# spiraldb/vortex

Hardware: AMD Instinct MI355X
Metric: decoded GB/s/GPU (device-resident) per encoding; % HBM roofline (higher is better)
Workload: dtype u32

## Files before the change

### vortex_amd/arrays.py

```python
from __future__ import annotations

import ctypes as C
from dataclasses import dataclass, field
from typing import Any, Optional, Sequence

import numpy as np

from . import _lib
from ._lib import DTYPE, ENC, PTYPE, PTYPES, VALIDITY, VortexGpuError

NP_OF_PTYPE = {"u8": np.uint8, "u16": np.uint16, "u32": np.uint32, "u64": np.uint64,
               "i8": np.int8, "i16": np.int16, "i32": np.int32, "i64": np.int64,
               "f16": np.float16, "f32": np.float32, "f64": np.float64}
PTYPE_OF_NP = {np.dtype(v): k for k, v in NP_OF_PTYPE.items()}


def ptype_width(p: str) -> int:
    return np.dtype(NP_OF_PTYPE[p]).itemsize


def unsigned_of(p: str) -> str:
    return "u" + p[1:] if p[0] == "i" else p


# ... 131 lines not shown
    return Array(ENC["ZIGZAG"], encoded.len, DTYPE["PRIMITIVE"], "i" + encoded.ptype[1:],
                 encoded.nullable, VALIDITY["NON_NULLABLE"], {}, [], [encoded])


def alp(encoded: Array, e: int, f: int, patches: Optional[Array] = None) -> Array:
    fp = {"i32": "f32", "i64": "f64"}.get(encoded.ptype)
    if fp is None:
        _bail("MismatchedTypes", f"ALP encoded child must be i32/i64, got {encoded.ptype}")
    return Array(ENC["ALP"], encoded.len, DTYPE["PRIMITIVE"], fp, encoded.nullable,
                 VALIDITY["NON_NULLABLE"], {"e": e, "f": f, "has_patches": patches is not None},
                 [], [encoded] + ([patches] if patches is not None else []))


def alp_rd(ptype: str, left_parts: Array, left_dict: Sequence[int], right_parts: Array,
           right_bit_width: int, exceptions: Optional[Array] = None) -> Array:
    if left_parts.len != right_parts.len:
        _bail("InvalidArgument", "left_parts and right_parts must be of same length")
    if left_parts.ptype[0] != "u":
        _bail("InvalidArgument", "left_parts dtype must be uint")
    if right_parts.nullable or right_parts.ptype[0] != "u":
        _bail("MismatchedTypes", "right_parts must be non-nullable uint")
    d = list(left_dict) + [0] * (8 - len(left_dict))
    return Array(ENC["ALP_RD"], left_parts.len, DTYPE["PRIMITIVE"], ptype, left_parts.nullable,
                 VALIDITY["NON_NULLABLE"],
                 {"right_bit_width": right_bit_width, "dict_len": len(left_dict), "dict": d,
                  "left_parts_ptype": PTYPE[left_parts.ptype], "has_exceptions": exceptions is not None},
                 [], [left_parts, right_parts] + ([exceptions] if exceptions is not None else []))


def dict_array(values: Array, codes: Array) -> Array:
    if codes.ptype[0] != "u" or codes.nullable:
        _bail("MismatchedTypes", f"non-nullable unsigned int, got {codes.ptype}")
    return Array(ENC["DICT"], codes.len, values.dtype, values.ptype, values.nullable,
                 VALIDITY["NON_NULLABLE"], {"codes_ptype": PTYPE[codes.ptype], "values_len": values.len},
                 [], [values, codes])


def delta(bases: Array, deltas: Array, offset: int = 0, length: Optional[int] = None,
          validity=None) -> Array:
    length = deltas.len - offset if length is None else length
    if offset >= 1024:
        _bail("InvalidArgument", f"offset must be less than 1024: {offset}")
    if offset + length > deltas.len:
        _bail("InvalidArgument", "offset + logical_len must be <= the size of deltas")
    if bases.ptype != deltas.ptype:
        _bail("InvalidArgument", "DeltaArray: bases and deltas must have the same dtype")
    lanes = 1024 // (8 * ptype_width(deltas.ptype))
    expect = (deltas.len // 1024) * lanes + (1 if deltas.len % 1024 else 0)
    if bases.len != expect:
        _bail("InvalidArgument", f"DeltaArray: bases.len() ({bases.len}) != expected_bases_len ({expect})")
    nullable = validity is not None
    vk, vchild = _validity_kind(nullable, validity)
    return Array(ENC["FL_DELTA"], length, DTYPE["PRIMITIVE"], deltas.ptype, nullable, vk,
                 {"deltas_len": deltas.len, "offset": offset}, [],
                 [bases, deltas] + ([vchild] if vchild is not None else []))


def run_end(ends: Array, values: Array, length: Optional[int] = None, offset: int = 0,
            validity=None) -> Array:
    if ends.ptype[0] not in "ui":
        _bail("InvalidArgument", "Run ends must be integers")
    if ends.encoding == ENC["PRIMITIVE"] and ends.len:
        ev = np.asarray(ends.buffers[0]).view(NP_OF_PTYPE[ends.ptype])
        if length is None:
            length = int(ev[ends.len - 1])
        if offset != 0 and int(ev[0]) <= offset:
            _bail("InvalidArgument", f"First run end {int(ev[0])} must be bigger than offset {offset}")
    elif length is None and ends.len == 0:
        length = 0
    if length is None:
        _bail("InvalidArgument", "length needed for compressed ends")
    nullable = validity is not None
    vk, vchild = _validity_kind(nullable, validity)
    return Array(ENC["RUN_END"], length, DTYPE["PRIMITIVE"], values.ptype, nullable, vk,
                 {"ends_ptype": PTYPE[ends.ptype], "num_runs": ends.len, "offset": offset}, [],
                 [ends, values] + ([vchild] if vchild is not None else []))


def bool_array(mask, validity=None, bit_offset: int = 0) -> Array:
    m = np.asarray(mask, dtype=bool)
    bits = np.packbits(np.concatenate([np.zeros(bit_offset, bool), m]), bitorder="little")
    nullable = validity is not None
    vk, vchild = _validity_kind(nullable, validity)
    return Array(ENC["BOOL"], len(m), DTYPE["BOOL"], "u8", nullable, vk, {"first_byte_bit_offset": bit_offset},
                 [bits], [vchild] if vchild is not None else [])


def byte_bool(mask, validity=None) -> Array:
    b = np.asarray(mask).astype(np.uint8)
    nullable = validity is not None
    vk, vchild = _validity_kind(nullable, validity)
    return Array(ENC["BYTE_BOOL"], len(b), DTYPE["BOOL"], "u8", nullable, vk, {}, [b],
                 [vchild] if vchild is not None else [])


def roaring_bool(bitmap, length: int) -> Array:
    b = np.ascontiguousarray(bitmap).view(np.uint8).reshape(-1)
    return Array(ENC["ROARING_BOOL"], length, DTYPE["BOOL"], "u8", False, VALIDITY["NON_NULLABLE"], {}, [b])


def run_end_bool(ends: Array, start: bool, length: Optional[int] = None, offset: int = 0, validity=None) -> Array:
    if ends.ptype[0] != "u":
        _bail("InvalidArgument", f"Ends array must be an unsigned integer type, got {ends.ptype}")
    if ends.len == 0:
        _bail("InvalidArgument", "Ends array must have at least one element")
    if length is None:
        length = int(np.asarray(ends.buffers[0])[ends.len - 1]) if ends.encoding == ENC["PRIMITIVE"] else None
        if length is None:
            _bail("InvalidArgument", "length needed for compressed ends")
    nullable = validity is not None
    vk, vchild = _validity_kind(nullable, validity)
    return Array(ENC["RUN_END_BOOL"], length, DTYPE["BOOL"], "u8", nullable, vk,
                 {"start": bool(start), "ends_ptype": PTYPE[ends.ptype], "num_runs": ends.len, "offset": offset},
                 [], [ends] + ([vchild] if vchild is not None else []))


def constant_bool(value: Optional[bool], length: int) -> Array:
    sc = bytes(16) if value is None else bytes([1 if value else 0]).ljust(16, b"\0")
    return Array(ENC["CONSTANT"], length, DTYPE["BOOL"], "u8", value is None, VALIDITY["NON_NULLABLE"],
                 {"is_null": value is None, "scalar": sc})


def sparse_bool(indices: Array, values: Array, length: int, indices_offset: int = 0, fill=None) -> Array:
    if values.dtype != DTYPE["BOOL"]:
        _bail("MismatchedTypes", "sparse_bool values must be a Bool array")
    fill_bytes = bytes(16) if fill is None else bytes([1 if fill else 0]).ljust(16, b"\0")
    return Array(ENC["SPARSE"], length, DTYPE["BOOL"], "u8", True, VALIDITY["NON_NULLABLE"],
                 {"indices_offset": indices_offset, "indices_len": indices.len,
                  "fill_is_null": fill is None, "fill": fill_bytes}, [], [indices, values])


def constant(value, length: int, ptype: str) -> Array:
    sc = bytes(16) if value is None else np.array([value], dtype=NP_OF_PTYPE[ptype]).tobytes().ljust(16, b"\0")
    return Array(ENC["CONSTANT"], length, DTYPE["PRIMITIVE"], ptype, value is None,
                 VALIDITY["NON_NULLABLE"], {"is_null": value is None, "scalar": sc})


def chunked(chunks: Sequence[Array]) -> Array:
    if not chunks:
        _bail("InvalidArgument", "chunked needs at least one chunk for a dtype")
    d0 = (chunks[0].dtype, chunks[0].ptype)
    for c in chunks:
        if (c.dtype, c.ptype) != d0:
            _bail("MismatchedTypes", "Chunks must have the same dtype")
    offs = np.zeros(len(chunks) + 1, dtype=np.uint64)
    offs[1:] = np.cumsum([c.len for c in chunks])
    return Array(ENC["CHUNKED"], int(offs[-1]), chunks[0].dtype, chunks[0].ptype,
                 any(c.nullable for c in chunks), VALIDITY["NON_NULLABLE"],
                 {"nchunks": len(chunks)}, [], [primitive(offs)] + list(chunks))


def varbin(offsets: Array, data: Array, utf8: bool = True, validity=None) -> Array:
    nullable = validity is not None
    vk, vchild = _validity_kind(nullable, validity)
    return Array(ENC["VARBIN"], offsets.len - 1, DTYPE["UTF8" if utf8 else "BINARY"], "u8", nullable,
                 vk, {"offsets_ptype": PTYPE[offsets.ptype], "bytes_len": data.len}, [],
                 [offsets, data] + ([vchild] if vchild is not None else []))


def varbinview(views, buffers: Sequence, utf8: bool = True, validity=None) -> Array:
    v = np.ascontiguousarray(views, dtype=np.uint8).reshape(-1)
    if v.size % 16:
        _bail("InvalidArgument", "views must be a multiple of 16 bytes")
    bufs = [np.ascontiguousarray(b, dtype=np.uint8).reshape(-1) for b in buffers]
    if any(b.size >= 2 ** 32 for b in bufs):
        _bail("InvalidArgument", "buffer must be within 32-bit range")
    nullable = validity is not None
    vk, vchild = _validity_kind(nullable, validity)
    return Array(ENC["VARBINVIEW"], v.size // 16, DTYPE["UTF8" if utf8 else "BINARY"], "u8", nullable, vk,
                 {"n_buffers": len(bufs)}, [],
                 [primitive(v)] + [primitive(b) for b in bufs] + ([vchild] if vchild is not None else []))


def fsst(symbols: Array, symbol_lengths: Array, codes: Array, uncompressed_lengths: Array,
         utf8: bool = True) -> Array:
    if symbols.len > 255:
        _bail("InvalidArgument", "symbols array must have length <= 255")
    if symbols.len != symbol_lengths.len:
        _bail("InvalidArgument", "symbols and symbol_lengths arrays must have same length")
    if uncompressed_lengths.len != codes.len:
        _bail("InvalidArgument", "uncompressed_lengths must be same len as codes")
    if codes.encoding != ENC["VARBIN"]:
        _bail("InvalidArgument", "codes array must be VarBin")
    return Array(ENC["FSST"], codes.len, DTYPE["UTF8" if utf8 else "BINARY"], "u8", codes.nullable,
                 VALIDITY["NON_NULLABLE"],
                 {"symbols_len": symbols.len, "codes_nullable": codes.nullable,
                  "uncompressed_lengths_ptype": PTYPE[uncompressed_lengths.ptype]}, [],
                 [symbols, symbol_lengths, codes, uncompressed_lengths])


def _fill_meta(m: _lib.VxgMeta, a: Array) -> None:
    md = a.meta
    e = a.encoding
    if e == ENC["FL_BITPACKED"]:
        m.bitpacked.bit_width, m.bitpacked.has_patches, m.bitpacked.offset = (
            md["bit_width"], int(md["has_patches"]), md["offset"])
    elif e == ENC["FL_FOR"]:
        m.for_.reference, m.for_.shift = md["reference"], md["shift"]
    elif e == ENC["FL_DELTA"]:
        m.delta.deltas_len, m.delta.offset = md["deltas_len"], md["offset"]
    elif e == ENC["ALP"]:
        m.alp.e, m.alp.f, m.alp.has_patches = md["e"], md["f"], int(md["has_patches"])
    elif e == ENC["ALP_RD"]:
        m.alprd.right_bit_width = md["right_bit_width"]
        m.alprd.dict_len = md["dict_len"]
        m.alprd.left_parts_ptype = md["left_parts_ptype"]
        m.alprd.has_exceptions = int(md["has_exceptions"])
        for i, v in enumerate(md["dict"]):
            m.alprd.dict[i] = v
    elif e == ENC["DICT"]:
        m.dict.codes_ptype, m.dict.values_len = md["codes_ptype"], md["values_len"]
    elif e == ENC["FSST"]:
        m.fsst.symbols_len = md["symbols_len"]
        m.fsst.codes_nullable = int(md["codes_nullable"])
        m.fsst.uncompressed_lengths_ptype = md["uncompressed_lengths_ptype"]
    elif e == ENC["RUN_END"]:
        m.runend.ends_ptype, m.runend.num_runs, m.runend.offset = (
            md["ends_ptype"], md["num_runs"], md["offset"])
    elif e == ENC["SPARSE"]:
        m.sparse.indices_offset = md["indices_offset"]
        m.sparse.indices_len = md["indices_len"]
        m.sparse.fill_is_null = int(md["fill_is_null"])
        for i, b in enumerate(md["fill"][:16]):
            m.sparse.fill[i] = b
    elif e == ENC["CONSTANT"]:
        m.constant.is_null = int(md["is_null"])
        for i, b in enumerate(md["scalar"][:16]):
            m.constant.scalar[i] = b
    elif e == ENC["CHUNKED"]:
        m.chunked.nchunks = md["nchunks"]
    elif e == ENC["VARBIN"]:
        m.varbin.offsets_ptype, m.varbin.bytes_len = md["offsets_ptype"], md["bytes_len"]
    elif e == ENC["BOOL"]:
        m.boolean.first_byte_bit_offset = md.get("first_byte_bit_offset", 0)
    elif e == ENC["RUN_END_BOOL"]:
        m.runendbool.start, m.runendbool.ends_ptype = int(md["start"]), md["ends_ptype"]
        m.runendbool.num_runs, m.runendbool.offset = md["num_runs"], md["offset"]
    elif e == ENC["VARBINVIEW"]:
        m.varbinview.n_buffers = md["n_buffers"]


def _buf_ptr(b) -> tuple[int, int]:
    import torch
    if not isinstance(b, torch.Tensor) or not b.is_cuda:
        raise VortexError(3, "array buffers must be device tensors: call Array.to(device) first")
    return b.data_ptr(), b.numel() * b.element_size()


def flatten(a: Array, keep: list) -> _lib.VxgArray:
    node = _lib.VxgArray()
    node.encoding = a.encoding
    node.dtype = a.dtype
    node.ptype = PTYPE[a.ptype]
    node.nullable = int(a.nullable)
    node.validity = a.validity
    node.len = a.len
    _fill_meta(node.meta, a)
    if a.buffers:
        bufs = (_lib.VxgBuffer * len(a.buffers))()
        for i, b in enumerate(a.buffers):
            bufs[i].ptr, bufs[i].len = _buf_ptr(b)
            keep.append(b)
        keep.append(bufs)
        node.buffers = C.cast(bufs, C.POINTER(_lib.VxgBuffer))
        node.n_buffers = len(a.buffers)
    if a.children:
        kids = (_lib.VxgArray * len(a.children))()
        for i, c in enumerate(a.children):
            kids[i] = flatten(c, keep)
        keep.append(kids)
        node.children = C.cast(kids, C.POINTER(_lib.VxgArray))
        node.n_children = len(a.children)
    return node


class Context:

    def __init__(self, device: int = 0):
        self.lib = _lib.gpu_lib()
        self.device = device
        h = C.c_void_p()
        _lib.check(self.lib.vxg_open(device, C.byref(h)))
        self.handle = h

    def close(self):
        if self.handle:
            self.lib.vxg_close(self.handle)
            self.handle = None

    def __del__(self):
        try:
            self.close()
        except Exception:
            pass

    def stream_ptr(self):
        import torch
        return C.c_void_p(torch.cuda.current_stream(self.device).cuda_stream)

    def sync(self):
        _lib.check(self.lib.vxg_stream_sync(self.handle, self.stream_ptr()))

    _OPTIONS = {"k1w_min_groups": _lib.OPT_K1W_MIN_GROUPS, "k1w_bpw": _lib.OPT_K1W_BPW,
                "k1_wave": _lib.OPT_K1_WAVE}

    def set_option(self, name: str, value: int):
        _lib.check(self.lib.vxg_set_option(self.handle, self._OPTIONS[name], int(value)))

    def get_option(self, name: str) -> int:
        v = C.c_int64()
        _lib.check(self.lib.vxg_get_option(self.handle, self._OPTIONS[name], C.byref(v)))
        return v.value

    def launch_stats(self, reset: bool = False) -> dict:
        st = _lib.VxgLaunchStats()
        _lib.check(self.lib.vxg_get_launch_stats(self.handle, C.byref(st), int(reset)))
        return {f: getattr(st, f) for f, _ in st._fields_}


@dataclass
class Canonical:
    kind: str
    len: int
    ptype: str
    values: Any = None
    views: Any = None
    data: Any = None
    validity: Any = None
    data_buffers: Any = None
    binary: bool = False
    info: Any = None

    def to_arrow(self):
        import pyarrow as pa
        validity = None if self.validity is None else pa.py_buffer(self.validity.cpu().numpy()[: (self.len + 7) // 8].copy())
        nulls = -1 if validity is not None else 0
        if self.kind == "primitive":
            t = {"u8": pa.uint8(), "u16": pa.uint16(), "u32": pa.uint32(), "u64": pa.uint64(), "i8": pa.int8(),
                 "i16": pa.int16(), "i32": pa.int32(), "i64": pa.int64(), "f16": pa.float16(), "f32": pa.float32(),
                 "f64": pa.float64()}[self.ptype]
            return pa.Array.from_buffers(t, self.len, [validity, pa.py_buffer(self.values.cpu().numpy().copy())],
                                         null_count=nulls)
        if self.kind == "bool":
            bits = self.values.cpu().numpy()[: (self.len + 7) // 8].copy()
            return pa.Array.from_buffers(pa.bool_(), self.len, [validity, pa.py_buffer(bits)], null_count=nulls)
        data = self.data.cpu().numpy()
        bufs = [pa.py_buffer(data[o: o + n].copy()) for o, n in self.data_buffers]
        views = pa.py_buffer(self.views.cpu().numpy()[: 16 * self.len].copy())
        return pa.Array.from_buffers(pa.binary_view() if self.binary else pa.string_view(), self.len,
                                     [validity, views] + bufs, null_count=nulls)

    def numpy(self):
        if self.kind == "primitive":
            return self.values.cpu().numpy().view(NP_OF_PTYPE[self.ptype])
        if self.kind == "bool":
            return np.unpackbits(self.values.cpu().numpy(), bitorder="little")[: self.len].astype(bool)
        return self.views.cpu().numpy().reshape(-1, 16), self.data.cpu().numpy()

    def buffers(self):
        d = self.data.cpu().numpy()
        return [d[o: o + n] for o, n in self.data_buffers]

    def validity_mask(self):
        if self.validity is None:
            return None
        bits = self.validity.cpu().numpy()
        return np.unpackbits(bits, bitorder="little")[: self.len].astype(bool)


def _kind(a: Array) -> str:
    return {DTYPE["PRIMITIVE"]: "primitive", DTYPE["BOOL"]: "bool"}.get(a.dtype, "varbinview")


def canonicalize(a: Array, ctx: Context, out_values=None, sync: bool = True) -> Canonical:
    import torch
    keep: list = []
    node = flatten(a, keep)
    dev = torch.device("cuda", ctx.device)
    vb, db, nb = C.c_uint64(), C.c_uint64(), C.c_uint32()
    cap = 256
    while True:
        table = (_lib.VxgDataBuffer * cap)()
        st = ctx.lib.vxg_canonical_layout(ctx.handle, C.byref(node), C.byref(vb), C.byref(db), table, cap,
                                          C.byref(nb))
        if st == 3 and cap < (1 << 24):
            cap *= 16
            continue
        _lib.check(st)
        break
    out = _lib.VxgCanonical()
    res = Canonical(_kind(a), a.len, a.ptype, binary=a.dtype == DTYPE["BINARY"])
    nbits = ((a.len + 31) // 32) * 4
    valid_t = torch.empty(max(nbits, 4), dtype=torch.uint8, device=dev) if a.nullable else None
    if a.dtype in (DTYPE["PRIMITIVE"], DTYPE["BOOL"]):
        vals = out_values if out_values is not None else torch.empty(max(vb.value, 16), dtype=torch.uint8, device=dev)
        out.values = vals.data_ptr()
        res.values = vals[: vb.value]
    else:
        views = torch.empty(max(vb.value, 16), dtype=torch.uint8, device=dev)
        data = torch.empty(db.value + 16, dtype=torch.uint8, device=dev)
        out.views, out.data = views.data_ptr(), data.data_ptr()
        out.data_bytes = db.value
        out.data_buffers, out.n_data_buffers, out.data_buffers_cap = table, nb.value, nb.value
        res.views, res.data = views[: vb.value], data[: db.value]
        res.data_buffers = [(int(table[i].offset), int(table[i].len)) for i in range(nb.value)]
    if valid_t is not None:
        out.validity = valid_t.data_ptr()
    _lib.check(ctx.lib.vxg_canonicalize(ctx.handle, C.byref(node), C.byref(out), ctx.stream_ptr()))
    if out.validity:
        if valid_t is None or out.validity != valid_t.data_ptr():
            raise VortexError(7, "engine allocated validity for a non-nullable dtype")
        res.validity = valid_t[: (a.len + 7) // 8]
    if sync:
        ctx.sync()
    return res


def take(a: Array, indices, ctx: Context, sync: bool = True) -> Canonical:
    import torch
    keep: list = []
    node = flatten(a, keep)
    dev = torch.device("cuda", ctx.device)
    if isinstance(indices, torch.Tensor):
        it = indices.to(dev)
        tmap = {torch.uint8: "u8", torch.int8: "i8", torch.int16: "i16", torch.int32: "i32", torch.int64: "i64"}
        for name, p in (("uint16", "u16"), ("uint32", "u32"), ("uint64", "u64")):
            if hasattr(torch, name):
                tmap[getattr(torch, name)] = p
        if it.dtype not in tmap:
            raise VortexError(3, f"take: indices must be integers, got {it.dtype}")
        ip = tmap[it.dtype]
    else:
        ia = np.ascontiguousarray(indices)
        if ia.dtype not in PTYPE_OF_NP or ia.dtype.kind not in "iu":
            raise VortexError(3, f"take: indices must be integers, got {ia.dtype}")
        ip = PTYPE_OF_NP[ia.dtype]
        it = torch.from_numpy(ia.view(np.uint8).copy()).to(dev)
    n = int(it.numel() if isinstance(indices, torch.Tensor) else np.asarray(indices).size)
    out = _lib.VxgCanonical()
    w = ptype_width(a.ptype)
    vals = torch.empty(max(n * w, 16), dtype=torch.uint8, device=dev)
    out.values = vals.data_ptr()
    vt = torch.empty(((n + 31) // 32) * 4 + 4, dtype=torch.uint8, device=dev) if a.nullable else None
    if vt is not None:
        out.validity = vt.data_ptr()
    _lib.check(ctx.lib.vxg_take_array(ctx.handle, C.byref(node), PTYPE[ip], C.c_void_p(it.data_ptr()), n,
                                      C.byref(out), ctx.stream_ptr()))
    res = Canonical("primitive", n, a.ptype, values=vals[: n * w])
    if out.validity:
        if vt is None or out.validity != vt.data_ptr():
            raise VortexError(7, "engine allocated validity for a non-nullable dtype")
        res.validity = vt[: (n + 7) // 8]
    if sync:
        ctx.sync()
    return res


def filter(a: Array, predicate: Array, ctx: Context) -> Canonical:
    import torch
    keep: list = []
    node = flatten(a, keep)
    pnode = flatten(predicate, keep)
    dev = torch.device("cuda", ctx.device)
    n = a.len
    out = _lib.VxgCanonical()
    kind = _kind(a)
    if kind == "primitive":
        buf = torch.empty(max(n * ptype_width(a.ptype), 16), dtype=torch.uint8, device=dev)
        out.values = buf.data_ptr()
    elif kind == "bool":
        buf = torch.empty(((n + 31) // 32) * 4 + 4, dtype=torch.uint8, device=dev)
        out.values = buf.data_ptr()
    else:
        buf = torch.empty(max(16 * n, 16), dtype=torch.uint8, device=dev)
        out.views = buf.data_ptr()
    vt = torch.empty(((n + 31) // 32) * 4 + 4, dtype=torch.uint8, device=dev) if a.nullable else None
    if vt is not None:
        out.validity = vt.data_ptr()
    table = (_lib.VxgDataBuffer * 1)()
    out.data_buffers, out.data_buffers_cap = table, 1
    _lib.check(ctx.lib.vxg_filter_array(ctx.handle, C.byref(node), C.byref(pnode), C.byref(out), ctx.stream_ptr()))
    k = int(out.len)
    res = Canonical(kind, k, a.ptype, binary=a.dtype == DTYPE["BINARY"])
    if kind == "primitive":
        res.values = buf[: k * ptype_width(a.ptype)]
    elif kind == "bool":
        res.values = buf[: ((k + 31) // 32) * 4]
    else:
        res.views = buf[: 16 * k]
        hb = int(out.data_bytes)
        heap = torch.empty(hb + 16, dtype=torch.uint8, device=dev)
        if out.data:
            _lib.check(ctx.lib.vxg_memcpy_d2d(ctx.handle, C.c_void_p(heap.data_ptr()), C.c_void_p(out.data), hb,
                                              ctx.stream_ptr()))
            ctx.sync()
            _lib.check(ctx.lib.vxg_free(ctx.handle, C.c_void_p(out.data)))
        res.data = heap[:hb]
        res.data_buffers = [(0, hb)]
    if out.validity:
        if vt is None or out.validity != vt.data_ptr():
            raise VortexError(7, "engine allocated validity for a non-nullable dtype")
        res.validity = vt[: (k + 7) // 8]
    ctx.sync()
    return res


def compare(a: Array, op: str, scalar, ctx: Context, null_as_false: bool = False, sync: bool = True,
            out_values=None, out_validity=None) -> Canonical:
    import torch
    if op not in _lib.CMP_OP:
        raise VortexError(3, f"compare: unknown operator {op!r}")
    keep: list = []
    node = flatten(a, keep)
    dev = torch.device("cuda", ctx.device)
    nbytes = ((a.len + 63) // 64) * 8
    vals = out_values if out_values is not None else torch.empty(max(nbytes, 8), dtype=torch.uint8, device=dev)
    out = _lib.VxgCanonical()
    out.values = vals.data_ptr()
    vt = None
    if a.nullable and not null_as_false:
        vt = out_validity if out_validity is not None else torch.empty(max(nbytes, 8), dtype=torch.uint8, device=dev)
        out.validity = vt.data_ptr()
    flags = _lib.CMP_NULL_AS_FALSE if null_as_false else 0
    if a.dtype in (DTYPE["UTF8"], DTYPE["BINARY"]) and isinstance(scalar, (bytes, bytearray, memoryview, str)):
        sc = scalar.encode("utf-8") if isinstance(scalar, str) else bytes(scalar)
        sbuf = (C.c_uint8 * max(len(sc), 1)).from_buffer_copy(sc.ljust(1, b"\0"))
        info = _lib.VxgCompareBytesInfo()
        _lib.check(ctx.lib.vxg_compare_bytes(ctx.handle, C.byref(node), _lib.CMP_OP[op], sbuf, len(sc), flags,
                                             C.byref(out), C.byref(info), ctx.stream_ptr()))
    else:
        sc = np.array([scalar]).astype(NP_OF_PTYPE[a.ptype]).tobytes() if a.dtype == DTYPE["PRIMITIVE"] else bytes(8)
        sbuf = (C.c_uint8 * 8)(*sc.ljust(8, b"\0")[:8])
        info = _lib.VxgCompareInfo()
        _lib.check(ctx.lib.vxg_compare_scalar(ctx.handle, C.byref(node), _lib.CMP_OP[op], sbuf, flags, C.byref(out),
                                              C.byref(info), ctx.stream_ptr()))
    res = Canonical("bool", a.len, a.ptype, values=vals[:nbytes],
                    info={f: int(getattr(info, f)) for f, _ in info._fields_})
    if out.validity:
        if vt is None or out.validity != vt.data_ptr():
            raise VortexError(7, "engine allocated validity for a non-nullable dtype")
        res.validity = vt[:nbytes]
    if sync:
        ctx.sync()
    return res


def predicate_from(mask: Canonical) -> Array:
    if mask.kind != "bool":
        _bail("MismatchedTypes", "predicate_from needs a Bool canonical")
    if mask.validity is not None:
        _bail("InvalidArgument", "predicate must be non-nullable bool: compare with null_as_false=True")
    return Array(ENC["BOOL"], mask.len, DTYPE["BOOL"], "u8", False, VALIDITY["NON_NULLABLE"],
                 {"first_byte_bit_offset": 0}, [mask.values])


def _kind_of_node(node: _lib.VxgArray) -> str:
    return {DTYPE["PRIMITIVE"]: "primitive", DTYPE["BOOL"]: "bool"}.get(node.dtype, "varbinview")


def alloc_canonical(ctx: Context, node: _lib.VxgArray, keep: list, table_cap: int = 4096):
    import torch
    dev = torch.device("cuda", ctx.device)
    vb, db, nb = C.c_uint64(), C.c_uint64(), C.c_uint32()
    table = (_lib.VxgDataBuffer * table_cap)()
    _lib.check(ctx.lib.vxg_canonical_layout(ctx.handle, C.byref(node), C.byref(vb), C.byref(db), table,
                                            table_cap, C.byref(nb)))
    n = int(node.len)
    res = Canonical(_kind_of_node(node), n, PTYPES[node.ptype], binary=node.dtype == DTYPE["BINARY"])
    o = _lib.VxgCanonical()
    if node.dtype in (DTYPE["PRIMITIVE"], DTYPE["BOOL"]):
        vals = torch.empty(max(vb.value, 16), dtype=torch.uint8, device=dev)
        o.values = vals.data_ptr()
        res.values = vals[: vb.value]
    else:
        views = torch.empty(max(vb.value, 16), dtype=torch.uint8, device=dev)
        data = torch.empty(db.value + 16, dtype=torch.uint8, device=dev)
        o.views, o.data, o.data_bytes = views.data_ptr(), data.data_ptr(), db.value
        o.data_buffers, o.n_data_buffers, o.data_buffers_cap = table, nb.value, table_cap
        res.views, res.data = views[: vb.value], data[: db.value]
        res.data_buffers = [(int(table[k].offset), int(table[k].len)) for k in range(nb.value)]
        keep.append(table)
    if node.nullable:
        vt = torch.empty(((n + 31) // 32) * 4 + 4, dtype=torch.uint8, device=dev)
        o.validity = vt.data_ptr()
        res.validity = vt[: (n + 7) // 8]
    keep.append(res)
    return o, res


class Plan:

    def __init__(self, arrays: Sequence, ctx: Context, measure: bool = False):
        self.ctx = ctx
        self.keep: list = []
        n = len(arrays)
        self.nodes = (_lib.VxgArray * max(n, 1))()
        self.outs = (_lib.VxgCanonical * max(n, 1))()
        self.results = []
        for i, a in enumerate(arrays):
            self.nodes[i] = a if isinstance(a, _lib.VxgArray) else flatten(a, self.keep)
            o, res = alloc_canonical(ctx, self.nodes[i], self.keep)
            self.outs[i] = o
            self.results.append(res)
        h = C.c_void_p()
        flags = _lib.PLAN_MEASURE if measure else 0
        _lib.check(ctx.lib.vxg_plan_create_ex(ctx.handle, self.nodes, self.outs, n, flags, C.byref(h)))
        self.handle = h
# ... 32 lines not shown
```

### vortex_amd/csrc/capi.hip

```cpp
#include <algorithm>
#include <cstring>
#include <mutex>

#include "encode_gpu.hpp"
#include "planner.hpp"

namespace vxg {

const float kF10f[11] = {1.0f, 10.0f, 100.0f, 1000.0f, 10000.0f, 100000.0f, 1000000.0f,
                         10000000.0f, 100000000.0f, 1000000000.0f, 10000000000.0f};
const float kIF10f[11] = {1.0f, 0.1f, 0.01f, 0.001f, 0.0001f, 0.00001f, 0.000001f,
                          0.0000001f, 0.00000001f, 0.000000001f, 0.0000000001f};
const double kF10d[24] = {
    1.0, 10.0, 100.0, 1000.0, 10000.0, 100000.0, 1000000.0, 10000000.0, 100000000.0,
    1000000000.0, 10000000000.0, 100000000000.0, 1000000000000.0, 10000000000000.0,
    100000000000000.0, 1000000000000000.0, 10000000000000000.0, 100000000000000000.0,
    1000000000000000000.0, 10000000000000000000.0, 100000000000000000000.0,
    1000000000000000000000.0, 10000000000000000000000.0, 100000000000000000000000.0};
const double kIF10d[24] = {
    1.0, 0.1, 0.01, 0.001, 0.0001, 0.00001, 0.000001, 0.0000001, 0.00000001, 0.000000001,
    0.0000000001, 0.00000000001, 0.000000000001, 0.0000000000001, 0.00000000000001,
    0.000000000000001, 0.0000000000000001, 0.00000000000000001, 0.000000000000000001,
    0.0000000000000000001, 0.00000000000000000001, 0.000000000000000000001,
    0.0000000000000000000001, 0.00000000000000000000001};

static thread_local std::string g_last_error;

vxg_status set_error(vxg_status s, const std::string& msg) {
    if (s != VXG_OK) g_last_error = msg;
    return s;
}

vxg_status hip_check(hipError_t e, const char* what) {
    if (e == hipSuccess) return VXG_OK;
    return set_error(e == hipErrorOutOfMemory ? VXG_ERR_OUT_OF_MEMORY : VXG_ERR_HIP,
                     std::string(what) + ": " + hipGetErrorString(e));
}

thread_local Ctx* g_cur_ctx = nullptr;

Options default_options() {
    static const Options d = [] {
        Options o;
        o.k1w_min_groups = int64_t(env_int("VXG_K1W_MIN_GROUPS", INT64_MIN, INT64_MAX, o.k1w_min_groups));
        return o;
    }();
    return d;
}

vxg_status use_device(vxg_ctx* ctx) {
    if (!ctx) return set_error(VXG_ERR_INVALID_ARGUMENT, "null vxg_ctx");
    g_cur_ctx = &ctx->c;
    return hip_check(hipSetDevice(ctx->c.device), "hipSetDevice");
}

vxg_status status_of_err_word(uint32_t err) {
    if (err & kErrTakeOOB) return set_error(VXG_ERR_OUT_OF_BOUNDS, "take: index out of bounds");
    if (err & kErrPatchOOB) return set_error(VXG_ERR_OUT_OF_BOUNDS, "patch index out of bounds");
    if (err & kErrPatchOrder) return set_error(VXG_ERR_INVALID_ARGUMENT, "patch indices are not sorted");
    if (err & kErrRunEnd) return set_error(VXG_ERR_INVALID_ARGUMENT, "RunEnd ends do not cover the array");
    if (err & kErrFsst) return set_error(VXG_ERR_INVALID_ARGUMENT, "FSST codes do not decode to uncompressed_lengths");
    if (err & kErrRoaring) return set_error(VXG_ERR_INVALID_SERDE, "RoaringBool buffer is not a croaring Native bitmap");
    if (err & kErrVarBin) return set_error(VXG_ERR_INVALID_ARGUMENT, "VarBin offsets out of range of the bytes");
    if (err & kErrPlanSync)
        return set_error(VXG_ERR_ASSERTION_FAILED, "plan launch: in-grid pre-pass records never published "
                                                   "(overlapping replays of one plan?)");
    return set_error(VXG_ERR_ASSERTION_FAILED, "unknown device error bit");
}

}

using namespace vxg;

static vxg_status bitunpack_common(vxg_ctx* ctx, int T, unsigned W, unsigned offset, uint64_t len,
                                   const void* packed, uint64_t packed_bytes, Epi epi, int vw,
                                   UnpackArgs a, void* out, void* stream) {
    std::vector<K1Job> jobs(1);
    VXG_TRY(make_k1_job(T, W, offset, len, packed, packed_bytes, epi, vw, a, out, jobs[0]));
    return launch_k1_jobs(jobs, ctx->c.err_word, S(stream), nullptr, nullptr);
}

extern "C" {

int vxg_abi_version(void) { return VXG_ABI_VERSION; }

const char* vxg_last_error(void) { return g_last_error.c_str(); }

vxg_status vxg_open(int device, vxg_ctx** out) {
    if (!out) return set_error(VXG_ERR_INVALID_ARGUMENT, "null out");
    int n = 0;
    VXG_TRY(hip_check(hipGetDeviceCount(&n), "hipGetDeviceCount"));
    if (device < 0 || device >= n) return set_error(VXG_ERR_INVALID_ARGUMENT, "no such device");
    VXG_TRY(hip_check(hipSetDevice(device), "hipSetDevice"));
    auto* c = new vxg_ctx();
    c->c.device = device;
    c->c.opt = default_options();
    hipError_t e = hipMalloc(&c->c.err_word, 16);
    if (e == hipSuccess) e = hipMemset(c->c.err_word, 0, 16);
    if (e == hipSuccess) {
        hipMemPool_t pool;
        uint64_t keep = ~0ull;
        if (hipDeviceGetDefaultMemPool(&pool, device) == hipSuccess)
            (void)hipMemPoolSetAttribute(pool, hipMemPoolAttrReleaseThreshold, &keep);
    }
    if (e == hipSuccess) e = fsst_diag_init();
    if (e != hipSuccess) {
        vxg_close(c);
        return hip_check(e, "context setup");
    }
    *out = c;
    return VXG_OK;
}

vxg_status vxg_set_option(vxg_ctx* ctx, int option, int64_t value) {
    if (!ctx) return set_error(VXG_ERR_INVALID_ARGUMENT, "null vxg_ctx");
    Options& o = ctx->c.opt;
    switch (option) {
    case VXG_OPT_K1W_MIN_GROUPS:
        if (value < 0 || value > (int64_t(1) << 31)) return set_error(VXG_ERR_INVALID_ARGUMENT, "K1W_MIN_GROUPS out of range");
        o.k1w_min_groups = value;
        return VXG_OK;
    case VXG_OPT_K1W_BPW:
        if (value < 0 || value > 32) return set_error(VXG_ERR_INVALID_ARGUMENT, "K1W_BPW must be in [0, 32]");
        o.k1w_bpw = value;
        return VXG_OK;
    case VXG_OPT_K1_WAVE:
        if (value < -1 || value > 2) return set_error(VXG_ERR_INVALID_ARGUMENT, "K1_WAVE must be -1, 0, 1 or 2");
        o.k1_wave = value;
        return VXG_OK;
    }
    return set_error(VXG_ERR_INVALID_ARGUMENT, "unknown option " + std::to_string(option));
}

vxg_status vxg_get_option(vxg_ctx* ctx, int option, int64_t* value) {
    if (!ctx || !value) return set_error(VXG_ERR_INVALID_ARGUMENT, "null argument");
    const Options& o = ctx->c.opt;
    switch (option) {
    case VXG_OPT_K1W_MIN_GROUPS: *value = o.k1w_min_groups; return VXG_OK;
    case VXG_OPT_K1W_BPW: *value = o.k1w_bpw; return VXG_OK;
    case VXG_OPT_K1_WAVE: *value = o.k1_wave; return VXG_OK;
    }
    return set_error(VXG_ERR_INVALID_ARGUMENT, "unknown option " + std::to_string(option));
}

vxg_status vxg_get_launch_stats(vxg_ctx* ctx, vxg_launch_stats* out, int reset) {
    if (!ctx || !out) return set_error(VXG_ERR_INVALID_ARGUMENT, "null argument");
    std::lock_guard<std::mutex> lk(ctx->c.mu);
    const LaunchStats& st = ctx->c.st;
    *out = vxg_launch_stats{};
    out->k1w_launches = st.k1w_launches;
    out->k1w_last_groups = st.k1w_last_groups;
    out->k1w_last_bpw = st.k1w_last_bpw;
    out->k1w_min_bpw = st.k1w_min_bpw;
    out->k1w_max_bpw = st.k1w_max_bpw;
    out->k1w_last_bpw_max = st.k1w_last_bpw_max;
    if (reset) ctx->c.st = LaunchStats{};
    return VXG_OK;
}

vxg_status vxg_close(vxg_ctx* ctx) {
    if (!ctx) return VXG_OK;
    if (g_cur_ctx == &ctx->c) g_cur_ctx = nullptr;
    (void)hipSetDevice(ctx->c.device);
    (void)hipDeviceSynchronize();
    if (ctx->c.err_word) (void)hipFree(ctx->c.err_word);
    delete ctx;
    return VXG_OK;
}

vxg_status vxg_alloc(vxg_ctx* ctx, uint64_t bytes, void** dptr) {
    VXG_TRY(use_device(ctx));
    return hip_check(hipMalloc(dptr, bytes ? bytes : 16), "hipMalloc");
}

vxg_status vxg_free(vxg_ctx* ctx, void* dptr) {
    VXG_TRY(use_device(ctx));
    return hip_check(hipFree(dptr), "hipFree");
}

vxg_status vxg_host_alloc(vxg_ctx* ctx, uint64_t bytes, void** hptr) {
    VXG_TRY(use_device(ctx));
    return hip_check(hipHostMalloc(hptr, bytes ? bytes : 16, hipHostMallocDefault), "hipHostMalloc");
}

vxg_status vxg_host_free(vxg_ctx* ctx, void* hptr) {
    VXG_TRY(use_device(ctx));
    return hip_check(hipHostFree(hptr), "hipHostFree");
}

vxg_status vxg_memcpy_h2d(vxg_ctx* ctx, void* dst, const void* src, uint64_t bytes, void* stream) {
    VXG_TRY(use_device(ctx));
    return hip_check(hipMemcpyAsync(dst, src, bytes, hipMemcpyHostToDevice, S(stream)), "h2d");
}

vxg_status vxg_memcpy_d2h(vxg_ctx* ctx, void* dst, const void* src, uint64_t bytes, void* stream) {
    VXG_TRY(use_device(ctx));
    return hip_check(hipMemcpyAsync(dst, src, bytes, hipMemcpyDeviceToHost, S(stream)), "d2h");
}

vxg_status vxg_memcpy_d2d(vxg_ctx* ctx, void* dst, const void* src, uint64_t bytes, void* stream) {
    VXG_TRY(use_device(ctx));
    return hip_check(hipMemcpyAsync(dst, src, bytes, hipMemcpyDeviceToDevice, S(stream)), "d2d");
}

vxg_status vxg_stream_sync(vxg_ctx* ctx, void* stream) {
    VXG_TRY(use_device(ctx));
    VXG_TRY(hip_check(hipStreamSynchronize(S(stream)), "hipStreamSynchronize"));
    uint32_t err = 0;
    VXG_TRY(hip_check(hipMemcpy(&err, ctx->c.err_word, 4, hipMemcpyDeviceToHost), "error word readback"));
    if (err) {
        VXG_TRY(hip_check(hipMemset(ctx->c.err_word, 0, 4), "error word reset"));
        return status_of_err_word(err);
    }
    return VXG_OK;
}

vxg_status vxg_canonical_size(vxg_ctx* ctx, const vxg_array* a, uint64_t* values_bytes, uint64_t* data_bytes) {
    VXG_TRY(use_device(ctx));
    if (!a) return set_error(VXG_ERR_INVALID_ARGUMENT, "null array");
    Planner p(ctx, nullptr);
    uint64_t vb = 0, db = 0;
    VXG_TRY(p.canonical_size(*a, vb, db));
    if (values_bytes) *values_bytes = vb;
    if (data_bytes) *data_bytes = db;
    return VXG_OK;
}

vxg_status vxg_canonical_layout(vxg_ctx* ctx, const vxg_array* a, uint64_t* values_bytes, uint64_t* data_bytes,
                                vxg_data_buffer* bufs, uint32_t cap, uint32_t* n_bufs) {
    VXG_TRY(use_device(ctx));
    if (!a) return set_error(VXG_ERR_INVALID_ARGUMENT, "null array");
    Planner p(ctx, nullptr);
    uint64_t vb = 0, db = 0;
    uint32_t n = 0;
    if (is_string(*a)) {
        std::vector<vxg_data_buffer> v;
        VXG_TRY(p.string_layout(*a, v, db));
        vb = 16 * a->len;
        n = uint32_t(v.size());
        if (bufs && cap < n) return set_error(VXG_ERR_INVALID_ARGUMENT, "buffer table too small");
        if (bufs) std::copy(v.begin(), v.end(), bufs);
    } else {
        VXG_TRY(p.canonical_size(*a, vb, db));
    }
    if (values_bytes) *values_bytes = vb;
    if (data_bytes) *data_bytes = db;
    if (n_bufs) *n_bufs = n;
    return VXG_OK;
}

vxg_status vxg_canonicalize(vxg_ctx* ctx, const vxg_array* a, vxg_canonical* out, void* stream) {
    VXG_TRY(use_device(ctx));
    if (!a || !out) return set_error(VXG_ERR_INVALID_ARGUMENT, "null array/out");
    Planner p(ctx, S(stream));
    return p.canonical(*a, *out);
}

static int unsigned_T(int ptype) { return 8 * ptype_width(ptype); }

vxg_status vxg_bitunpack(vxg_ctx* ctx, int ptype, unsigned bit_width, unsigned offset, uint64_t len,
                         const void* packed, uint64_t packed_bytes, void* out, void* stream) {
    VXG_TRY(use_device(ctx));
    if (!ptype_is_int(ptype)) return set_error(VXG_ERR_MISMATCHED_TYPES, "BitPacked needs an integer ptype");
    return bitunpack_common(ctx, unsigned_T(ptype), bit_width, offset, len, packed, packed_bytes, Epi::Plain, 0,
                            UnpackArgs{}, out, stream);
}

vxg_status vxg_bitunpack_for(vxg_ctx* ctx, int ptype, unsigned bit_width, unsigned offset, uint64_t len,
                             const void* packed, uint64_t packed_bytes, uint64_t reference, unsigned shift,
                             int zigzag, void* out, void* stream) {
    VXG_TRY(use_device(ctx));
    if (!ptype_is_int(ptype)) return set_error(VXG_ERR_MISMATCHED_TYPES, "FoR needs an integer ptype");
    UnpackArgs a{};
    a.reference = reference;
    a.shift = shift;
    return bitunpack_common(ctx, unsigned_T(ptype), bit_width, offset, len, packed, packed_bytes,
                            zigzag ? Epi::ForZigZag : Epi::For, 0, a, out, stream);
}

vxg_status vxg_bitunpack_alp(vxg_ctx* ctx, int float_ptype, unsigned bit_width, unsigned offset, uint64_t len,
                             const void* packed, uint64_t packed_bytes, uint64_t for_reference,
                             unsigned for_shift, unsigned e, unsigned f, void* out, void* stream) {
    VXG_TRY(use_device(ctx));
    const bool f32 = float_ptype == VXG_F32;
    if (!f32 && float_ptype != VXG_F64) return set_error(VXG_ERR_MISMATCHED_TYPES, "ALP decodes to f32/f64");
    if ((f32 && (e > 10 || f > 10)) || (!f32 && (e > 23 || f > 23)))
        return set_error(VXG_ERR_INVALID_ARGUMENT, "ALP exponents out of range");
    UnpackArgs a{};
    a.reference = for_reference;
    a.shift = for_shift;
    a.alp_a = f32 ? double(kF10f[f]) : kF10d[f];
    a.alp_b = f32 ? double(kIF10f[e]) : kIF10d[e];
    return bitunpack_common(ctx, f32 ? 32 : 64, bit_width, offset, len, packed, packed_bytes,
                            f32 ? Epi::AlpF32 : Epi::AlpF64, 0, a, out, stream);
}

vxg_status vxg_bitunpack_dict(vxg_ctx* ctx, int codes_ptype, unsigned bit_width, unsigned offset, uint64_t len,
                              const void* packed, uint64_t packed_bytes, const void* dict_values,
                              uint64_t dict_len, unsigned value_width, void* out, void* stream) {
    VXG_TRY(use_device(ctx));
    if (!ptype_is_unsigned(codes_ptype)) return set_error(VXG_ERR_MISMATCHED_TYPES, "Dict codes must be unsigned");
    if (bit_width > unsigned(kDictFusedMaxW))
        return set_error(VXG_ERR_NOT_IMPLEMENTED, "fused dict decode supports code widths <= 16");
    UnpackArgs a{};
    a.dict = dict_values;
    a.dict_len = dict_len;
    return bitunpack_common(ctx, unsigned_T(codes_ptype), bit_width, offset, len, packed, packed_bytes, Epi::Dict,
                            int(value_width), a, out, stream);
}

vxg_status vxg_bitunpack_dict_chunks(vxg_ctx* ctx, int codes_ptype, unsigned bit_width, unsigned value_width,
                                     const vxg_dict_chunk* chunks_host, uint32_t n_chunks, void* stream) {
    VXG_TRY(use_device(ctx));
    if (!ptype_is_unsigned(codes_ptype)) return set_error(VXG_ERR_MISMATCHED_TYPES, "Dict codes must be unsigned");
    if (bit_width > unsigned(kDictFusedMaxW))
        return set_error(VXG_ERR_NOT_IMPLEMENTED, "fused dict decode supports code widths <= 16");
    std::vector<K1Job> jobs(n_chunks);
    for (uint32_t i = 0; i < n_chunks; i++) {
        const vxg_dict_chunk& c = chunks_host[i];
        if (c.n_blocks != (c.len + 1023) / 1024)
            return set_error(VXG_ERR_INVALID_ARGUMENT, "chunk n_blocks != ceil(len/1024)");
        UnpackArgs a{};
        a.dict = c.dict_values;
        a.dict_len = c.dict_len;
        VXG_TRY(make_k1_job(unsigned_T(codes_ptype), bit_width, 0, c.len, c.packed, c.n_blocks * 128ull * bit_width,
                            Epi::Dict, int(value_width), a, c.out, jobs[i]));
    }
    return launch_k1_jobs(jobs, ctx->c.err_word, S(stream), nullptr, nullptr);
}

vxg_status vxg_patch(vxg_ctx* ctx, int ptype, void* out, uint64_t out_len, int indices_ptype, const void* indices,
                     uint64_t indices_offset, const void* values, uint64_t n_patches, void* stream) {
    VXG_TRY(use_device(ctx));
    const int w = ptype_width(ptype);
    if (!w || !ptype_is_int(indices_ptype)) return set_error(VXG_ERR_INVALID_ARGUMENT, "bad ptype");
    UnpackArgs a{};
    a.err = ctx->c.err_word;
    IntCol ic{};
    ic.p = indices;
    ic.width = ptype_width(indices_ptype);
    ic.sgn = ptype_is_signed(indices_ptype);
    return launch_patch(0, ic, Epi::Plain, 8 * w, out, out_len, indices_offset, values, n_patches, a, S(stream));
}

vxg_status vxg_for_decode(vxg_ctx* ctx, int ptype, const void* in, uint64_t n, uint64_t reference,
                          unsigned shift, void* out, void* stream) {
    VXG_TRY(use_device(ctx));
    if (!ptype_is_int(ptype)) return set_error(VXG_ERR_MISMATCHED_TYPES, "FoR needs an integer ptype");
    return launch_for(ptype_width(ptype), in, n, reference, shift, false, out, S(stream));
}

vxg_status vxg_zigzag_decode(vxg_ctx* ctx, int out_ptype, const void* in, uint64_t n, void* out, void* stream) {
    VXG_TRY(use_device(ctx));
    if (!ptype_is_signed(out_ptype)) return set_error(VXG_ERR_MISMATCHED_TYPES, "ZigZag decodes to signed ints");
    return launch_zigzag(ptype_width(out_ptype), in, n, out, S(stream));
}

vxg_status vxg_alp_decode(vxg_ctx* ctx, int float_ptype, const void* encoded, uint64_t n, unsigned e, unsigned f,
                          void* out, void* stream) {
    VXG_TRY(use_device(ctx));
    const bool f32 = float_ptype == VXG_F32;
    if ((f32 && (e > 10 || f > 10)) || (!f32 && (e > 23 || f > 23)))
        return set_error(VXG_ERR_INVALID_ARGUMENT, "ALP exponents out of range");
    return launch_alp(float_ptype, encoded, n, f32 ? double(kF10f[f]) : kF10d[f],
                      f32 ? double(kIF10f[e]) : kIF10d[e], out, S(stream));
}

vxg_status vxg_alprd_decode(vxg_ctx* ctx, int float_ptype, const uint16_t* left_codes, const uint16_t* dict_host,
                            unsigned dict_len, unsigned right_bw, const void* right, uint64_t n,
                            const uint64_t* exc_pos, const uint16_t* exc_vals, uint64_t n_exc, void* out,
                            void* stream) {
    VXG_TRY(use_device(ctx));
    if (dict_len > 8) return set_error(VXG_ERR_INVALID_ARGUMENT, "ALP-RD dictionary holds at most 8 entries");
    return launch_alprd(float_ptype, left_codes, dict_host, dict_len, right_bw, right, n, exc_pos, 8, false, 0,
                        exc_vals, n_exc, out, ctx->c.err_word, S(stream));
}

vxg_status vxg_take(vxg_ctx* ctx, unsigned value_width, const void* values, uint64_t n_values, int codes_ptype,
                    const void* codes, uint64_t n, void* out, void* stream) {
    VXG_TRY(use_device(ctx));
    if (!ptype_is_unsigned(codes_ptype)) return set_error(VXG_ERR_MISMATCHED_TYPES, "take indices must be unsigned");
    return launch_take(int(value_width), values, n_values, ptype_width(codes_ptype), ptype_is_signed(codes_ptype), codes, n, out,
                       ctx->c.err_word, S(stream));
}

vxg_status vxg_delta_decode(vxg_ctx* ctx, int ptype, const void* bases, uint64_t n_bases, const void* deltas,
                            uint64_t n_deltas, uint64_t offset, uint64_t len, void* out, void* stream) {
    VXG_TRY(use_device(ctx));
    const int w = ptype_width(ptype);
    if (!ptype_is_unsigned(ptype)) return set_error(VXG_ERR_MISMATCHED_TYPES, "Delta decodes unsigned ints");
    const uint64_t lanes = 1024 / (8 * w);
    if (n_bases != (n_deltas / 1024) * lanes + (n_deltas % 1024 ? 1 : 0))
        return set_error(VXG_ERR_INVALID_ARGUMENT, "DeltaArray: bases.len() != expected_bases_len");
    if (offset + len > n_deltas) return set_error(VXG_ERR_INVALID_ARGUMENT, "offset + len > deltas len");
    return launch_delta(w, bases, deltas, n_deltas, offset, len, out, S(stream));
}

vxg_status vxg_runend_decode(vxg_ctx* ctx, unsigned value_width, const void* values, int ends_ptype,
                             const void* ends, uint64_t n_runs, uint64_t offset, uint64_t len, void* out,
                             void* stream) {
    VXG_TRY(use_device(ctx));
    if (!ptype_is_int(ends_ptype)) return set_error(VXG_ERR_MISMATCHED_TYPES, "RunEnd ends must be integers");
    RunEndChunk c{};
    c.ends.p = ends;
    c.ends.width = ptype_width(ends_ptype);
    c.ends.sgn = ptype_is_signed(ends_ptype);
    c.values.p = values;
    c.values.width = int(value_width);
    c.out = out;
    c.n_runs = n_runs;
    c.offset = offset;
    c.len = len;
    return launch_runend(int(value_width), c, ctx->c.err_word, S(stream));
}

vxg_status vxg_take_array(vxg_ctx* ctx, const vxg_array* a, int indices_ptype, const void* indices,
                          uint64_t n_indices, vxg_canonical* out, void* stream) {
    VXG_TRY(use_device(ctx));
    if (!a || !out || (n_indices && !indices)) return set_error(VXG_ERR_INVALID_ARGUMENT, "null array/indices/out");
    if (!ptype_is_int(indices_ptype)) return set_error(VXG_ERR_INVALID_ARGUMENT, "take indices must be integers");
    Planner p(ctx, S(stream));
    return p.take(*a, indices, ptype_width(indices_ptype), ptype_is_signed(indices_ptype), n_indices, *out);
}

vxg_status vxg_compare_scalar(vxg_ctx* ctx, const vxg_array* a, int op, const void* scalar_host, uint32_t flags,
                              vxg_canonical* out, vxg_compare_info* info, void* stream) {
    VXG_TRY(use_device(ctx));
    if (!a || !out || !scalar_host) return set_error(VXG_ERR_INVALID_ARGUMENT, "null array/scalar/out");
    uint64_t bits = 0;
    if (a->dtype == VXG_DTYPE_PRIMITIVE) std::memcpy(&bits, scalar_host, size_t(ptype_width(a->ptype)));
    vxg_compare_info ci{};
    Planner p(ctx, S(stream));
    void* const values_in = out->values;
    void* const validity_in = out->validity;
    const vxg_status st = p.compare(*a, op, bits, flags, *out, ci);
    if (info) *info = ci;
    if (st != VXG_OK) {
        if (out->values && out->values != values_in) (void)hipFree(out->values);
        if (out->validity && out->validity != validity_in) (void)hipFree(out->validity);
        out->values = values_in;
        out->validity = validity_in;
    }
    return st;
// ... 187 lines not shown
```

### vortex_amd/csrc/chunk_pack.hpp

```cpp
#pragma once

#include <algorithm>
#include <type_traits>

#include "vxg_internal.hpp"

namespace vxg {

template <class Tab, class It, class Entry, class Groups>
vxg_status pack_chunk_table(Tab& tab, It& it, It end, DevTables* dt, Entry entry, Groups groups_of, uint64_t* groups) {
    using E = std::remove_reference_t<decltype(tab.c[0])>;
    constexpr size_t cap = sizeof(tab.c) / sizeof(tab.c[0]);
    size_t take = 0;
    for (It k = it; k != end; ++k) take += entry(*k) != nullptr;
    E* cs = tab.c;
    if (dt && take > cap) {
        if (take > 0xFFFFFFFFull) return set_error(VXG_ERR_INVALID_ARGUMENT, "too many chunks");
        E* host;
        const vxg_status st = dt->table(take, &host, &tab.ext);
        if (st != VXG_OK) return st;
        if constexpr (requires { tab.host; }) tab.host = host;
        cs = host;
    } else {
        take = std::min(take, cap);
    }
    tab.n = 0;
    *groups = 0;
    for (; it != end && tab.n < take; ++it) {
        const E* e = entry(*it);
        if (!e) continue;
        E& c = cs[tab.n++];
        c = *e;
        c.first_group = *groups;
        *groups += groups_of(c);
    }
    while (it != end && !entry(*it)) ++it;
    if (*groups > 0xFFFFFFFFull) return set_error(VXG_ERR_INVALID_ARGUMENT, "array too long for one launch");
    return VXG_OK;
}

}
```

### vortex_amd/csrc/dict_rows.hip

```cpp
#include "fl_unpack_impl.hpp"

namespace vxg {

namespace {

constexpr int kRowsThreads = 256;
constexpr int kRowsMaxW = 16;

template <int VW> struct DVal;
template <> struct DVal<16> { using t = uint4; };

template <int T, int VW, int BPW, bool LDSD, bool EXT>
__global__ __launch_bounds__(kRowsThreads) void dict_rows_kernel(ChunkTable tab, unsigned W) {
    using E = typename Fl<T>::E;
    using V = typename DVal<VW>::t;
    constexpr unsigned LANES = 1024 / T;
    const uint64_t g = blockIdx.x;
    uint32_t ci;
    if constexpr (EXT) {
        ci = ext_chunk_index(tab.ext, tab.n, g, [](const ChunkDev& d) { return d.first_group; });
    } else {
        uint32_t lo = 0, hi = tab.n;
        while (hi - lo > 1) {
            const uint32_t mid = (lo + hi) >> 1;
            if (tab.c[mid].first_group <= g) lo = mid; else hi = mid;
        }
        ci = lo;
    }
    const ChunkDev& c = EXT ? tab.ext[ci] : tab.c[ci];
    __shared__ __attribute__((aligned(16))) E s_packed[BPW * 128 * kRowsMaxW / sizeof(E)];
    __shared__ __attribute__((aligned(16))) uint8_t s_dict[LDSD ? kDictLdsBytes : 16];
    const unsigned tid = threadIdx.x;
    const uint64_t blk0 = (g - c.first_group) * BPW;
    const unsigned nb = unsigned(c.n_blocks - blk0 < uint64_t(BPW) ? c.n_blocks - blk0 : uint64_t(BPW));
    const unsigned q16 = nb * 8 * W;
    for (unsigned q = tid; q < q16; q += kRowsThreads)
        reinterpret_cast<uint4*>(s_packed)[q] = reinterpret_cast<const uint4*>(c.packed + blk0 * (128ull * W))[q];
    const V* dict = static_cast<const V*>(c.dict);
    if constexpr (LDSD) {
        const unsigned n16 = unsigned((c.dict_len * VW + 15) / 16);
        for (unsigned q = tid; q < n16; q += kRowsThreads)
            reinterpret_cast<uint4*>(s_dict)[q] = static_cast<const uint4*>(c.dict)[q];
        dict = reinterpret_cast<const V*>(s_dict);
    }
    __syncthreads();
    V* __restrict__ out = static_cast<V*>(c.out);
    const RtRows<T> rows(W);
    bool oob = false;
    for (unsigned b = 0; b < nb; b++) {
        const E* __restrict__ pw = s_packed + b * (LANES * W);
        const int64_t base = int64_t((blk0 + b) * 1024) - int64_t(c.offset);
        const bool whole = base >= 0 && uint64_t(base) + 1024 <= c.len;
#pragma unroll
        for (unsigned k = 0; k < 4; k++) {
            const int64_t o = base + int64_t(k * kRowsThreads + tid);
            if (!whole && (o < 0 || uint64_t(o) >= c.len)) continue;
            const uint64_t code = W ? uint64_t(rows.get(pw, k)) : 0;
            const bool bad = code >= c.dict_len;
            oob |= bad;
            nt_store(out + o, dict[bad ? 0 : code]);
        }
    }
    if (oob) __hip_atomic_fetch_or(tab.err, kErrTakeOOB, __ATOMIC_RELAXED, __HIP_MEMORY_SCOPE_AGENT);
}

template <int T, int VW, int BPW, bool LDSD, bool EXT>
vxg_status launch_rows(ChunkTable tab, unsigned W, hipStream_t s) {
    ChunkDev* cs = tab.ext ? tab.host : tab.c;
    uint64_t groups = 0;
    for (uint32_t k = 0; k < tab.n; k++) {
        cs[k].first_group = groups;
        groups += (cs[k].n_blocks + BPW - 1) / BPW;
    }
    if (groups == 0) return VXG_OK;
    if (groups > 0xFFFFFFFFull) return set_error(VXG_ERR_INVALID_ARGUMENT, "array too long for one launch");
    hipLaunchKernelGGL((dict_rows_kernel<T, VW, BPW, LDSD, EXT>), dim3(unsigned(groups)), dim3(kRowsThreads), 0, s,
                       tab, W);
    return hip_check(hipGetLastError(), "dict_rows_kernel launch");
}

template <int T, int VW, int BPW>
vxg_status launch_rows_b(const ChunkTable& tab, unsigned W, bool lds, hipStream_t s) {
    if (tab.ext) return lds ? launch_rows<T, VW, BPW, true, true>(tab, W, s) : launch_rows<T, VW, BPW, false, true>(tab, W, s);
    return lds ? launch_rows<T, VW, BPW, true, false>(tab, W, s) : launch_rows<T, VW, BPW, false, false>(tab, W, s);
}

template <int T, int VW>
vxg_status launch_rows_t(const ChunkTable& tab, unsigned W, hipStream_t s) {
    const ChunkDev* cs = tab.ext ? tab.host : tab.c;
    bool lds = true;
    uint64_t max_dict = 0;
    for (uint32_t k = 0; k < tab.n; k++) {
        lds = lds && cs[k].dict_len * VW <= uint64_t(kDictLdsBytes) && (reinterpret_cast<uintptr_t>(cs[k].dict) & 15) == 0;
        max_dict = cs[k].dict_len * VW > max_dict ? cs[k].dict_len * VW : max_dict;
    }
    if (lds && max_dict > 1024) return launch_rows_b<T, VW, 8>(tab, W, lds, s);
    return launch_rows_b<T, VW, 1>(tab, W, lds, s);
}

}

vxg_status launch_dict_rows(int T, int W, const ChunkTable& tab, hipStream_t s) {
    if (W < 0 || W > kRowsMaxW || W > T) return VXG_ERR_NOT_IMPLEMENTED;
    const unsigned w = unsigned(W);
    switch (T) {
    case 8: return launch_rows_t<8, 16>(tab, w, s);
    case 16: return launch_rows_t<16, 16>(tab, w, s);
    case 32: return launch_rows_t<32, 16>(tab, w, s);
    case 64: return launch_rows_t<64, 16>(tab, w, s);
    }
    return VXG_ERR_NOT_IMPLEMENTED;
}

}
```

### vortex_amd/csrc/fl_unpack_impl.hpp

```cpp
#pragma once

#include <hip/hip_runtime.h>

#include <cstdint>
#include <cstdlib>
#include <type_traits>
#include <utility>

#include "vxg_internal.hpp"
#include "intcol.hpp"

namespace vxg {

template <int T> struct Fl;
template <> struct Fl<8> {
    using E = uint8_t;  using U = uint32_t;
    static constexpr uint32_t rep(uint32_t m) { return m * 0x01010101u; }
};
template <> struct Fl<16> {
    using E = uint16_t; using U = uint32_t;
    static constexpr uint32_t rep(uint32_t m) { return m * 0x00010001u; }
};
template <> struct Fl<32> {
    using E = uint32_t; using U = uint32_t;
// ... 284 lines not shown
    constexpr int WLO = W > 0 ? (R0 * W) / T : 0;
    constexpr int WHI = W > 0 ? (R1 * W - 1) / T : 0;
    Vec16<T> p[NW];
    if constexpr (W > 0) {
#pragma unroll
        for (int w = WLO; w <= WHI && w < W; w++) p[w] = load16<T>(blk_packed + 128 * w + 16 * t);
    }
    bool oob = false;
    if (full)
        process_rows_part<T, W, EPI, VW, NT, S, Q, true>(p, t * EPV, out, out_base, len, ep, oob,
                                                         std::make_integer_sequence<int, T / S>{});
    else
        process_rows_part<T, W, EPI, VW, NT, S, Q, false>(p, t * EPV, out, out_base, len, ep, oob,
                                                          std::make_integer_sequence<int, T / S>{});
    if constexpr (EPI == Epi::Dict)
        if (oob) __hip_atomic_fetch_or(ep.err, kErrTakeOOB, __ATOMIC_RELAXED, __HIP_MEMORY_SCOPE_AGENT);
}

constexpr int kDictLdsBytes = 16 * 1024;

template <int VW>
__device__ __forceinline__ void stage_dict(uint8_t* s_dict, const void* dict, uint64_t dict_len) {
    const int n16 = int((dict_len * VW + 15) / 16);
    for (int q = threadIdx.x; q < n16; q += blockDim.x)
        reinterpret_cast<uint4*>(s_dict)[q] = static_cast<const uint4*>(dict)[q];
    __syncthreads();
}

template <int T, int W, Epi EPI, int VW, bool LDSD, int S>
__device__ __forceinline__ void unpack_chunk(const ChunkDev& c, uint64_t g, uint32_t* err) {
    using O = typename EpiOut<T, EPI, VW>::type;
    constexpr int BPG = 32 / S;
    const uint64_t blk = (g - c.first_group) * BPG + ((threadIdx.x >> 3) % BPG);
    const int t = int(threadIdx.x & 7);
    EpiParams ep;
    ep.reference = c.reference;
    ep.shift = c.shift;
    ep.alp_a = c.alp_a;
    ep.alp_b = c.alp_b;
    ep.dict = c.dict;
    ep.dict_len = c.dict_len;
    ep.err = err;
    if constexpr (LDSD) {
        __shared__ __attribute__((aligned(16))) uint8_t s_dict[kDictLdsBytes];
        stage_dict<VW>(s_dict, c.dict, c.dict_len);
        ep.dict = s_dict;
        ep.dict_lds = true;
    }
    if (blk >= c.n_blocks) return;
    const int64_t out_base = int64_t(blk * 1024) - int64_t(c.offset);
    const bool full =
        c.offset == 0 && (blk + 1) * 1024 <= c.len && (reinterpret_cast<uintptr_t>(c.out) & 15) == 0;
    const uint8_t* bp = c.packed + blk * (128 * W);
    if constexpr (S == 1) {
        unpack_block<T, W, EPI, VW, kOutNT>(bp, t, static_cast<O*>(c.out), out_base, full, c.len, ep);
    } else {
        static_assert(S == 4, "row split 1 or 4");
        switch (threadIdx.x >> 6) {
        case 0: unpack_block_part<T, W, EPI, VW, kOutNT, 4, 0>(bp, t, static_cast<O*>(c.out), out_base, full, c.len, ep); break;
        case 1: unpack_block_part<T, W, EPI, VW, kOutNT, 4, 1>(bp, t, static_cast<O*>(c.out), out_base, full, c.len, ep); break;
        case 2: unpack_block_part<T, W, EPI, VW, kOutNT, 4, 2>(bp, t, static_cast<O*>(c.out), out_base, full, c.len, ep); break;
        default: unpack_block_part<T, W, EPI, VW, kOutNT, 4, 3>(bp, t, static_cast<O*>(c.out), out_base, full, c.len, ep); break;
        }
    }
}

constexpr int kw_bpw(int W, bool lds_dict = false) {
    const int b = ((lds_dict ? 16 : 32) * 1024) / (128 * (W > 0 ? W : 1));
    const int b4 = (b / 4) * 4;
    return b4 < 4 ? 4 : (b4 > 32 ? 32 : b4);
}

template <int T>
__device__ __forceinline__ int kw_row(int q) {
    constexpr int P = T / 8;
    const int s = q / P, f = (q % P) * (64 / T);
    const int o = ((f & 1) << 2) | (f & 2) | (f >> 2);
    return o * 8 + s;
}

template <typename U>
__device__ __forceinline__ U kw_mask(int n) {
    return n >= int(8 * sizeof(U)) ? ~U(0) : ((U(1) << n) - U(1));
}

template <int T, int W>
__device__ __forceinline__ Vec16<T> kw_extract(const uint8_t* blk, int r, int t) {
    using U = typename Fl<T>::U;
    constexpr int NV = Vec16<T>::NV;
    Vec16<T> v;
    if constexpr (W == 0) {
#pragma unroll
        for (int k = 0; k < NV; k++) v.w[k] = 0;
    } else {
        const int start = r * W, w0 = start / T, sh = start % T;
        const Vec16<T> lo = load16<T>(blk + w0 * 128 + 16 * t);
        if constexpr (W == T) {
            v = lo;
        } else {
            const Vec16<T> hi = load16<T>(blk + (w0 + 1) * 128 + 16 * t);
            const int cur = T - sh;
            const int nlo = cur < W ? cur : W, nhi = W - nlo;
            const U mlo = Fl<T>::rep(kw_mask<U>(nlo)), mhi = Fl<T>::rep(kw_mask<U>(nhi));
            const int hs = cur & (int(8 * sizeof(U)) - 1);
#pragma unroll
            for (int k = 0; k < NV; k++) v.w[k] = ((lo.w[k] >> sh) & mlo) | ((hi.w[k] & mhi) << hs);
        }
    }
    return v;
}

template <int T, int W, Epi EPI, int VW, int NT>
__device__ __forceinline__ void kw_block(const uint8_t* pk, int gq, int t, typename EpiOut<T, EPI, VW>::type* __restrict__ out,
                                         int64_t out_base, bool full, uint64_t len, const EpiParams& ep, bool& oob) {
    using E = typename Fl<T>::E;
    using O = typename EpiOut<T, EPI, VW>::type;
    constexpr int EPV = 16 / int(sizeof(E));
#pragma unroll
    for (int k = 0; k < T / 8; k++) {
        const int q = 8 * k + gq;
        const Vec16<T> v = kw_extract<T, W>(pk, kw_row<T>(q), t);
        const int idx = q * (1024 / T) + t * EPV;
        if (full) {
            O* dst = out + (out_base + idx);
            if constexpr (EPI == Epi::Plain) {
                store_bytes<16, NT>(reinterpret_cast<uint8_t*>(dst), v.w);
            } else {
                O o[EPV];
#pragma unroll
                for (int j = 0; j < EPV; j++) o[j] = apply_epi<T, EPI, VW>(v.elem(j), ep, oob);
                store_bytes<EPV * int(sizeof(O)), NT>(reinterpret_cast<uint8_t*>(dst), o);
            }
        } else {
#pragma unroll
            for (int j = 0; j < EPV; j++) {
                const int64_t o = out_base + idx + j;
                if (o >= 0 && uint64_t(o) < len) gstore(out + o, apply_epi<T, EPI, VW>(v.elem(j), ep, oob));
            }
        }
    }
}

template <int W, bool LDSD>
constexpr int kw_packed_lds() {
    return (W > 0 ? kw_bpw(W, LDSD) * 128 * W : 0) + 128;
}

__device__ __forceinline__ uint64_t patch_lower_bound(const PatchCol& pc, uint64_t x, uint32_t* s_cnt) {
    uint64_t lo = 0, hi = pc.n;
    while (lo < hi) {
        const uint64_t step = (hi - lo + 255) / 256;
        const uint64_t i = lo + uint64_t(threadIdx.x) * step;
        const bool below = i < hi && uint64_t(intcol_get(pc.idx, i)) - pc.idx_off < x;
        const uint32_t cw = uint32_t(__popcll(__ballot(below)));
        if ((threadIdx.x & 63) == 0) s_cnt[threadIdx.x >> 6] = cw;
        __syncthreads();
        const uint64_t cnt = uint64_t(s_cnt[0]) + s_cnt[1] + s_cnt[2] + s_cnt[3];
        __syncthreads();
        if (cnt == 0) {
            hi = lo;
        } else {
            const uint64_t nhi = lo + cnt * step;
            lo = lo + (cnt - 1) * step + 1;
            hi = nhi < hi ? nhi : hi;
        }
    }
    return lo;
}

template <int T, int W, Epi EPI, int VW, bool LDSD>
__device__ __forceinline__ void unpack_chunk_w(const ChunkDev& c, uint64_t g, uint32_t* err, const PatchCol& pc,
                                               uint32_t bpw_rt) {
    using O = typename EpiOut<T, EPI, VW>::type;
    constexpr int BPW_MAX = kw_bpw(W, LDSD);
    const int BPW = bpw_rt ? int(bpw_rt) : BPW_MAX;
    extern __shared__ __attribute__((aligned(16))) uint8_t k1w_lds[];
    uint8_t* const s_pk = k1w_lds;
    EpiParams ep;
    ep.reference = c.reference;
    ep.shift = c.shift;
    ep.alp_a = c.alp_a;
    ep.alp_b = c.alp_b;
    ep.dict = c.dict;
    ep.dict_len = c.dict_len;
    ep.err = err;
    if constexpr (LDSD) {
        uint8_t* const s_dict = k1w_lds + kw_packed_lds<W, LDSD>();
        stage_dict<VW>(s_dict, c.dict, c.dict_len);
        ep.dict = s_dict;
        ep.dict_lds = true;
    }
    const uint64_t blk0 = (g - c.first_group) * BPW;
    const int nb = c.n_blocks - blk0 < uint64_t(BPW) ? int(c.n_blocks - blk0) : BPW;
    uint32_t* const s_pscr = reinterpret_cast<uint32_t*>(k1w_lds + (W > 0 ? BPW * 128 * W : 0));
    const bool patched = pc.n != 0;
    uint64_t olo = 0, ohi = 0, pbase = 0, pw0 = 0, pw1 = 0;
    uint32_t psh = 0;
    O pval{};
    if (patched) {
        const uint64_t s0 = blk0 * 1024, s1 = (blk0 + uint64_t(nb)) * 1024;
        olo = s0 > c.offset ? s0 - c.offset : 0;
        ohi = s1 - c.offset < c.len ? s1 - c.offset : c.len;
        const uint64_t guess = uint64_t(double(olo) * double(pc.n) / double(c.len));
        pbase = guess > 128 ? guess - 128 : 0;
        if (pbase + 256 > pc.n) pbase = pc.n > 256 ? pc.n - 256 : 0;
        const uint64_t i0 = pbase + threadIdx.x, i = i0 < pc.n ? i0 : pc.n - 1;
        const uint64_t* ip = static_cast<const uint64_t*>(pc.idx.p);
        uint64_t a0 = i, a1 = i;
        if (pc.idx.packed) {
            const uint64_t g2 = i + pc.idx.offset;
            const uint32_t e = uint32_t(g2 & 1023), lane = e % 16, s = e >> 7;
            const uint32_t fl = ((e & 127) - lane) >> 4;
            const uint32_t row = (((fl & 1) << 2) | (fl & 2) | (fl >> 2)) * 8 + s;
            const uint32_t start = __umul24(row, pc.idx.W), word = start / 64;
            psh = start % 64;
            const uint64_t blk = (g2 >> 10) * (16ull * pc.idx.W);
            a0 = blk + 16ull * word + lane;
            a1 = blk + 16ull * (word + 1 < pc.idx.W ? word + 1 : word) + lane;
        }
        pw0 = ip[a0];
        pw1 = ip[a1];
        pval = static_cast<const O*>(pc.vals)[i];
    }
    if constexpr (W > 0) {
        using u32x4 = unsigned int __attribute__((ext_vector_type(4)));
        const gptr<const u32x4> src = (gptr<const u32x4>)(c.packed + blk0 * (128 * W));
#if VXG_K1W_BURST
        constexpr int NQ = BPW_MAX * 8 * W, PQ = (NQ + 255) / 256;
        if (nb == BPW_MAX) {
            u32x4 v[PQ];
#pragma unroll
            for (int p = 0; p < PQ; p++) {
                const int q = int(threadIdx.x) + 256 * p;
                v[p] = __builtin_nontemporal_load(src + (q < NQ ? q : NQ - 1));
            }
#pragma unroll
            for (int p = 0; p < PQ; p++) {
                const int q = int(threadIdx.x) + 256 * p;
                if (q < NQ) reinterpret_cast<uint4*>(s_pk)[q] = make_uint4(v[p][0], v[p][1], v[p][2], v[p][3]);
            }
        } else
#endif
        for (int q = threadIdx.x; q < nb * 8 * W; q += 256) {
            const u32x4 v = __builtin_nontemporal_load(src + q);
            reinterpret_cast<uint4*>(s_pk)[q] = make_uint4(v[0], v[1], v[2], v[3]);
        }
    }
    __syncthreads();
    const int wave = threadIdx.x >> 6, lane = threadIdx.x & 63, gq = lane >> 3, t = lane & 7;
    O* const out = static_cast<O*>(c.out);
    const bool aligned = (reinterpret_cast<uintptr_t>(c.out) & 15) == 0;
    bool oob = false;
    const int PER = (BPW + 3) / 4;
    for (int j = 0; j < PER; j++) {
        const int b = wave * PER + j;
        if (b >= nb) break;
        const uint64_t blk = blk0 + b;
        const int64_t out_base = int64_t(blk * 1024) - int64_t(c.offset);
        const bool full = c.offset == 0 && (blk + 1) * 1024 <= c.len && aligned;
        kw_block<T, W, EPI, VW, kOutNT>(s_pk + b * 128 * W, gq, t, out, out_base, full, c.len, ep, oob);
    }
    if constexpr (EPI == Epi::Dict)
        if (oob) __hip_atomic_fetch_or(err, kErrTakeOOB, __ATOMIC_RELAXED, __HIP_MEMORY_SCOPE_AGENT);
    if (patched) {
        asm volatile("" : "+v"(pw0), "+v"(pw1));
        uint64_t pkey = pw0;
        if (pc.idx.packed) {
            const uint64_t mask = pc.idx.W >= 64 ? ~0ull : ((1ull << pc.idx.W) - 1);
            const uint64_t v = pc.idx.W ? ((psh ? (pw0 >> psh) | (pw1 << (64 - psh)) : pw0) & mask) : 0;
            pkey = (v << pc.idx.shift) + pc.idx.reference;
        }
        const bool valid = pbase + threadIdx.x < pc.n;
        pkey = valid ? pkey - pc.idx_off : ~0ull;
        const bool pin = pkey >= olo && pkey < ohi;
        if (threadIdx.x == 0) s_pscr[0] = pbase == 0 || pkey < olo;
        if (threadIdx.x == 255) s_pscr[1] = pbase + 256 >= pc.n || pkey >= ohi;
        const uint64_t nk = __shfl_down(pkey, 1, 64);
        if ((threadIdx.x & 63) != 63 && pbase + threadIdx.x + 1 < pc.n && nk < pkey)
            __hip_atomic_fetch_or(err, kErrPatchOrder, __ATOMIC_RELAXED, __HIP_MEMORY_SCOPE_AGENT);
        if (g == c.first_group && threadIdx.x == 0) {
            const uint64_t k0 = uint64_t(intcol_get(pc.idx, 0)) - pc.idx_off;
            const uint64_t k1 = uint64_t(intcol_get(pc.idx, pc.n - 1)) - pc.idx_off;
            if (k0 >= c.len || k1 >= c.len)
                __hip_atomic_fetch_or(err, kErrPatchOOB, __ATOMIC_RELAXED, __HIP_MEMORY_SCOPE_AGENT);
        }
        __builtin_amdgcn_s_waitcnt(0);
        __syncthreads();
        if (s_pscr[0] && s_pscr[1]) {
            if (pin) gstore(out + pkey, pval);
        } else {
            const uint64_t ps = patch_lower_bound(pc, olo, s_pscr + 4);
            const uint64_t pe = patch_lower_bound(pc, ohi, s_pscr + 4);
            bool bad = false;
            for (uint64_t i = ps + threadIdx.x; i < pe; i += 256) {
                const uint64_t key = uint64_t(intcol_get(pc.idx, i)) - pc.idx_off;
                if (key >= olo && key < ohi) gstore(out + key, gload(static_cast<const O*>(pc.vals) + i));
                else bad = true;
            }
            if (bad) __hip_atomic_fetch_or(err, kErrPatchOrder, __ATOMIC_RELAXED, __HIP_MEMORY_SCOPE_AGENT);
        }
    }
}

template <int T, int W, Epi EPI, int VW, bool LDSD, bool EXT>
__global__ __launch_bounds__(256) void fl_unpack_w_kernel(ChunkTable tab) {
    const uint64_t g = blockIdx.x;
    if constexpr (EXT) {
        const ChunkDev& c =
            tab.ext[ext_chunk_index(tab.ext, tab.n, g, [](const ChunkDev& d) { return d.first_group; })];
        unpack_chunk_w<T, W, EPI, VW, LDSD>(c, g, tab.err, PatchCol{}, tab.bpw);
    } else {
        uint32_t lo = 0, hi = tab.n;
        while (hi - lo > 1) {
            const uint32_t mid = (lo + hi) >> 1;
            if (tab.c[mid].first_group <= g) lo = mid; else hi = mid;
        }
        unpack_chunk_w<T, W, EPI, VW, LDSD>(tab.c[lo], g, tab.err, tab.patch, tab.bpw);
    }
}

template <int T, int W, Epi EPI, int VW, bool LDSD = false, int S = 1, bool EXT = false>
__global__ __launch_bounds__(256) void fl_unpack_kernel(ChunkTable tab) {
    const uint64_t g = blockIdx.x;
    if constexpr (EXT) {
        const ChunkDev& c =
            tab.ext[ext_chunk_index(tab.ext, tab.n, g, [](const ChunkDev& d) { return d.first_group; })];
        unpack_chunk<T, W, EPI, VW, LDSD, S>(c, g, tab.err);
    } else {
        uint32_t lo = 0, hi = tab.n;
        while (hi - lo > 1) {
            const uint32_t mid = (lo + hi) >> 1;
            if (tab.c[mid].first_group <= g) lo = mid; else hi = mid;
        }
        unpack_chunk<T, W, EPI, VW, LDSD, S>(tab.c[lo], g, tab.err);
    }
}


inline int k1w_pick_bpw(uint64_t blocks, int bpw_max, int64_t min_groups, int64_t forced) {
    if (forced > 0) return int(forced < bpw_max ? forced : bpw_max);
    if (min_groups <= 0 || blocks >= uint64_t(min_groups) * uint64_t(bpw_max)) return bpw_max;
    const uint64_t b = blocks / uint64_t(min_groups);
    const int bpw = int(b < 4 ? 4 : (b / 4) * 4);
    return bpw > bpw_max ? bpw_max : bpw;
}

template <int T, int W, Epi EPI, int VW, bool LDSD, bool EXT>
vxg_status launch_w(ChunkTable tab, hipStream_t s) {
    constexpr int BPW_MAX = kw_bpw(W, LDSD);
    ChunkDev* cs = tab.ext ? tab.host : tab.c;
    uint64_t blocks = 0;
    for (uint32_t k = 0; k < tab.n; k++) blocks += cs[k].n_blocks;
    const Options o = cur_options();
    const int BPW = k1w_pick_bpw(blocks, BPW_MAX, o.k1w_min_groups, o.k1w_bpw);
    tab.bpw = uint32_t(BPW);
    uint64_t groups = 0, dict_bytes = 0;
    for (uint32_t k = 0; k < tab.n; k++) {
        cs[k].first_group = groups;
        groups += (cs[k].n_blocks + BPW - 1) / BPW;
        const uint64_t db = (cs[k].dict_len * uint64_t(VW > 0 ? VW : 1) + 15) & ~15ull;
        dict_bytes = db > dict_bytes ? db : dict_bytes;
    }
    if (groups == 0) return VXG_OK;
    if (groups > 0xFFFFFFFFull) return set_error(VXG_ERR_INVALID_ARGUMENT, "array too long for one launch");
    const size_t shm = LDSD ? size_t(kw_packed_lds<W, LDSD>()) + size_t(dict_bytes)
                            : size_t(W > 0 ? BPW * 128 * W : 0) + 128;
    hipLaunchKernelGGL((fl_unpack_w_kernel<T, W, EPI, VW, LDSD, EXT>), dim3(unsigned(groups)), dim3(256), shm, s, tab);
    note_k1w_launch(uint32_t(BPW), uint32_t(BPW_MAX), groups);
    return hip_check(hipGetLastError(), "fl_unpack_w_kernel launch");
}


template <int T, int W, Epi EPI, int VW, bool LDSD, int S, bool EXT = false>
vxg_status launch_s(ChunkTable tab, hipStream_t s) {
    ChunkDev* cs = tab.ext ? tab.host : tab.c;
    uint64_t groups = 0;
    for (uint32_t k = 0; k < tab.n; k++) {
        cs[k].first_group = groups;
        groups += (cs[k].n_blocks + (32 / S) - 1) / (32 / S);
    }
    if (groups == 0) return VXG_OK;
    if (groups > 0xFFFFFFFFull) return set_error(VXG_ERR_INVALID_ARGUMENT, "array too long for one launch");
    hipLaunchKernelGGL((fl_unpack_kernel<T, W, EPI, VW, LDSD, S, EXT>), dim3(unsigned(groups)), dim3(256), 0, s, tab);
    return hip_check(hipGetLastError(), "fl_unpack_kernel launch");
}

template <int T, int W, Epi EPI, int VW>
vxg_status launch_one(const ChunkTable& tab, uint64_t groups32, hipStream_t s) {
    constexpr bool kSplit = (T == 32 || T == 64) && W > 0;
    bool lds_ok = false;
    if constexpr (EPI == Epi::Dict) {
        const ChunkDev* cs = tab.ext ? tab.host : tab.c;
        lds_ok = true;
        for (uint32_t k = 0; k < tab.n; k++)
            lds_ok = lds_ok && cs[k].dict_len * VW <= uint64_t(kDictLdsBytes) &&
                     (reinterpret_cast<uintptr_t>(cs[k].dict) & 15) == 0;
    }
    const K1Choice c = k1_choose(T, W, EPI, tab.ext != nullptr, groups32, lds_ok, k1_wave_mode(), split_below_groups());
    const bool wave = c.kind == K1Kind::Wave;
    if (tab.patch.n && (!wave || tab.ext))
        return set_error(VXG_ERR_INVALID_ARGUMENT, "internal: patches handed to a K1 launch that does not write them");
    if (c.kind == K1Kind::None) return VXG_OK;
    if (tab.ext) {
        if (wave) {
            if constexpr (EPI == Epi::Dict) {
                if (c.lds) return launch_w<T, W, EPI, VW, true, true>(tab, s);
            }
            return launch_w<T, W, EPI, VW, false, true>(tab, s);
        }
        constexpr int SX = kSplit ? 4 : 1;
        if constexpr (EPI == Epi::Dict) {
            if (c.lds) return launch_s<T, W, EPI, VW, true, SX, true>(tab, s);
        }
        return launch_s<T, W, EPI, VW, false, SX, true>(tab, s);
    }
    if constexpr (kSplit) {
        if (c.kind == K1Kind::RegSplit)
            return c.lds ? launch_s<T, W, EPI, VW, true, 4>(tab, s) : launch_s<T, W, EPI, VW, false, 4>(tab, s);
    }
    if (wave) {
        if constexpr (EPI == Epi::Dict) {
            if (c.lds) return launch_w<T, W, EPI, VW, true, false>(tab, s);
        }
        return launch_w<T, W, EPI, VW, false, false>(tab, s);
    }
    if constexpr (EPI == Epi::Dict) {
        if (c.lds) return launch_s<T, W, EPI, VW, true, 1>(tab, s);
    }
    return launch_s<T, W, EPI, VW, false, 1>(tab, s);
}

template <int T, Epi EPI, int VW, int... Ws>
vxg_status dispatch_w_impl(int W, const ChunkTable& tab, uint64_t groups, hipStream_t s,
                           std::integer_sequence<int, Ws...>) {
    using Fn = vxg_status (*)(const ChunkTable&, uint64_t, hipStream_t);
    static constexpr Fn table[] = {&launch_one<T, Ws, EPI, VW>...};
    if (W < 0 || W >= int(sizeof...(Ws))) return VXG_ERR_NOT_IMPLEMENTED;
    return table[W](tab, groups, s);
}

template <int T, Epi EPI, int VW, int WMAX>
vxg_status dispatch_w(int W, const ChunkTable& tab, uint64_t groups, hipStream_t s) {
    return dispatch_w_impl<T, EPI, VW>(W, tab, groups, s, std::make_integer_sequence<int, WMAX + 1>{});
}

}
```

### vortex_amd/csrc/kernels.hip

```cpp
#include "fl_unpack_impl.hpp"
#include "intcol.hpp"
#include "runend_runs.hpp"

namespace vxg {

namespace {

constexpr int kBlock = 256;

inline unsigned grid_for(uint64_t n_threads) {
    uint64_t g = (n_threads + kBlock - 1) / kBlock;
    const uint64_t cap = 256ull * 8 * 16;
    if (g > cap) g = cap;
    if (g == 0) g = 1;
    return unsigned(g);
}

__device__ __forceinline__ uint64_t load_uint(const void* p, int width, bool sgn, uint64_t i) {
    switch (width) {
    case 1: return sgn ? uint64_t(int64_t(gload(static_cast<const int8_t*>(p) + i))) : gload(static_cast<const uint8_t*>(p) + i);
    case 2: return sgn ? uint64_t(int64_t(gload(static_cast<const int16_t*>(p) + i))) : gload(static_cast<const uint16_t*>(p) + i);
    case 4: return sgn ? uint64_t(int64_t(gload(static_cast<const int32_t*>(p) + i))) : gload(static_cast<const uint32_t*>(p) + i);
    default: return gload(static_cast<const uint64_t*>(p) + i);
    }
// ... 467 lines not shown
        lo = nlo;
        hi = nhi;
    }
    const uint64_t idx = lo + uint64_t(lane);
    const bool gt = idx < hi ? load_uint(ends, ew, false, idx) - offset > j : false;
    const unsigned long long bm = __ballot(gt);
    return bm ? lo + uint64_t(__ffsll(bm) - 1) : hi;
}

__device__ __forceinline__ uint64_t runend_locate(const void* ends, int ew, uint64_t offset, uint64_t n_runs,
                                                  uint64_t len, uint64_t j) {
    const int lane = threadIdx.x & 63;
    constexpr uint64_t S = 64;
    const uint64_t guess = uint64_t(double(j) / double(len) * double(n_runs));
    const uint64_t base = guess > 32 * S ? guess - 32 * S : 0;
    if (base >= n_runs) return runend_first_gt_in(ends, ew, offset, 0, n_runs, j);
    const uint64_t idx = base + S * uint64_t(lane);
    const bool gt = idx < n_runs ? load_uint(ends, ew, false, idx) - offset > j : true;
    const unsigned long long bm = __ballot(gt);
    if (bm & 1ull) return base == 0 ? 0 : runend_first_gt_in(ends, ew, offset, 0, base + 1, j);
    if (bm == 0) return runend_first_gt_in(ends, ew, offset, base + 63 * S + 1, n_runs, j);
    const int k = __ffsll(bm) - 1;
    const uint64_t lo = base + S * uint64_t(k - 1) + 1;
    const uint64_t hi = base + S * uint64_t(k) < n_runs ? base + S * uint64_t(k) + 1 : n_runs;
    return runend_first_gt_in(ends, ew, offset, lo, hi, j);
}

template <typename V>
__global__ __launch_bounds__(kBlock) void runend_chunks_kernel(RunEndTable tab) {
    constexpr int SPAN = int(kRunEndSpan), PER = SPAN / kBlock;
    __shared__ uint32_t s_head[SPAN];
    __shared__ uint32_t s_wmax[kBlock / 64];
    __shared__ uint64_t s_r0;
    __shared__ int s_bad;
    const uint64_t g = blockIdx.x;
    RunEndChunk c;
    if (tab.ext) {
        c = tab.ext[ext_chunk_index(tab.ext, tab.n, g, [](RunEndChunk const& d) { return d.first_group; })];
    } else {
        uint32_t lo = 0, hi = tab.n;
        while (hi - lo > 1) {
            const uint32_t mid = (lo + hi) >> 1;
            if (tab.c[mid].first_group <= g) lo = mid; else hi = mid;
        }
        c = tab.c[lo];
    }
    const V* __restrict__ values = static_cast<const V*>(c.values.p);
    const void* ends = c.ends.p;
    V* __restrict__ out = static_cast<V*>(c.out);
    const int ew = c.ends.width, tid = threadIdx.x;
    const uint64_t j0 = (g - c.first_group) * SPAN;
    const int jn = int(c.len - j0 < uint64_t(SPAN) ? c.len - j0 : uint64_t(SPAN));
    const uint64_t jend = j0 + uint64_t(jn);
    if (tid < 64) {
        const uint64_t r0 = runend_locate(ends, ew, c.offset, c.n_runs, c.len, j0);
        if (tid == 0) s_r0 = r0;
    } else if (tid == 64) {
        s_bad = c.n_runs == 0 || load_uint(ends, ew, false, c.n_runs - 1) - c.offset < c.len;
    }
#pragma unroll
    for (int k = 0; k < PER; k++) s_head[tid + k * kBlock] = 0;
    __syncthreads();
    if (s_bad) {
        if (tid == 0) __hip_atomic_fetch_or(tab.err, kErrRunEnd, __ATOMIC_RELAXED, __HIP_MEMORY_SCOPE_AGENT);
        return;
    }
    const uint64_t r0 = s_r0;
    constexpr int Q = 4;
    for (uint64_t rb = r0;; rb += uint64_t(Q) * kBlock) {
        uint64_t st[Q];
#pragma unroll
        for (int q = 0; q < Q; q++) {
            const uint64_t r = rb + uint64_t(q) * kBlock + uint64_t(tid);
            st[q] = r + 1 < c.n_runs ? load_uint(ends, ew, false, r) - c.offset : ~0ull;
        }
#pragma unroll
        for (int q = 0; q < Q; q++)
            if (st[q] < jend) s_head[st[q] - j0] = uint32_t(rb + uint64_t(q) * kBlock + uint64_t(tid) + 1 - r0);
        if (!__syncthreads_or(st[Q - 1] < jend)) break;
    }
    __syncthreads();
    uint32_t v[PER];
    uint32_t m = 0;
#pragma unroll
    for (int k = 0; k < PER; k++) {
        m = max(m, s_head[tid * PER + k]);
        v[k] = m;
    }
    uint32_t x = m;
#pragma unroll
    for (int d = 1; d < 64; d <<= 1) {
        const uint32_t y = __shfl_up(x, d, 64);
        if ((tid & 63) >= d) x = max(x, y);
    }
    if ((tid & 63) == 63) s_wmax[tid >> 6] = x;
    __syncthreads();
    uint32_t before = __shfl_up(x, 1, 64);
    if ((tid & 63) == 0) before = 0;
#pragma unroll
    for (int w = 0; w < kBlock / 64; w++)
        if (w < (tid >> 6)) before = max(before, s_wmax[w]);
#pragma unroll
    for (int k = 0; k < PER; k++) s_head[tid * PER + k] = max(v[k], before);
    __syncthreads();
    for (int i = tid; i < jn; i += kBlock) nt_store(out + j0 + i, gload(values + r0 + s_head[i]));
}

template <typename V>
__global__ __launch_bounds__(kBlock) void runend_runs_kernel(RunEndTable tab) {
    __shared__ __attribute__((aligned(16))) uint8_t lds[runs_lds_bytes<V>()];
    const uint64_t g = blockIdx.x;
    RunEndChunk c;
    if (tab.ext) {
        c = tab.ext[ext_chunk_index(tab.ext, tab.n, g, [](RunEndChunk const& d) { return d.first_group; })];
    } else {
        uint32_t lo = 0, hi = tab.n;
        while (hi - lo > 1) {
            const uint32_t mid = (lo + hi) >> 1;
            if (tab.c[mid].first_group <= g) lo = mid; else hi = mid;
        }
        c = tab.c[lo];
    }
    runend_runs_body<V>(c, g, tab.err, lds);
}

vxg_status launch_runend_runs(int value_width, const RunEndTable& t, uint64_t groups, hipStream_t s) {
    if (groups == 0) return VXG_OK;
    switch (value_width) {
#define RR_CASE(W)                                                                                                \
    case W:                                                                                                       \
        hipLaunchKernelGGL((runend_runs_kernel<typename UInt<W>::t>), dim3(unsigned(groups)), dim3(kBlock), 0, s, t); \
        break;
        RR_CASE(1) RR_CASE(2) RR_CASE(4) RR_CASE(8) RR_CASE(16)
#undef RR_CASE
    default: return VXG_ERR_INVALID_ARGUMENT;
    }
    return hip_check(hipGetLastError(), "runend_runs_kernel");
}

vxg_status launch_runend_chunks(int value_width, const RunEndTable& t, uint64_t groups, hipStream_t s) {
    if (groups == 0) return VXG_OK;
    switch (value_width) {
#define RE_CASE(W)                                                                                  \
    case W:                                                                                         \
        hipLaunchKernelGGL((runend_chunks_kernel<typename UInt<W>::t>), dim3(unsigned(groups)), dim3(kBlock), 0, s, t); \
        break;
        RE_CASE(1) RE_CASE(2) RE_CASE(4) RE_CASE(8) RE_CASE(16)
#undef RE_CASE
    default: return VXG_ERR_INVALID_ARGUMENT;
    }
    return hip_check(hipGetLastError(), "runend_chunks_kernel");
}

vxg_status launch_runend(int value_width, const RunEndChunk& chunk, uint32_t* err, hipStream_t s) {
    if (chunk.len == 0) return VXG_OK;
    if (chunk.n_runs == 0) return set_error(VXG_ERR_INVALID_ARGUMENT, "RunEnd with len > 0 has no runs");
    RunEndTable t{};
    t.err = err;
    t.n = 1;
    t.c[0] = chunk;
    t.c[0].first_group = 0;
    if (chunk.len <= kRunEndShortRun * chunk.n_runs)
        return launch_runend_runs(value_width, t, (chunk.n_runs + kRunEndRunsPerGroup - 1) / kRunEndRunsPerGroup, s);
    if (chunk.ends.packed || chunk.values.packed)
        return set_error(VXG_ERR_INVALID_ARGUMENT, "long-run RunEnd expansion reads plain ends/values");
    return launch_runend_chunks(value_width, t, (chunk.len + kRunEndSpan - 1) / kRunEndSpan, s);
}

template <typename V>
__global__ __launch_bounds__(kBlock) void fill_kernel(V v, uint64_t n, V* __restrict__ out) {
    const uint64_t stride = uint64_t(gridDim.x) * blockDim.x;
    for (uint64_t i = uint64_t(blockIdx.x) * blockDim.x + threadIdx.x; i < n; i += stride) nt_store(out + i, v);
}

vxg_status launch_fill(int value_width, const uint8_t* scalar16, uint64_t n, void* out, hipStream_t s) {
    if (n == 0) return VXG_OK;
    const unsigned g = grid_for(n);
    switch (value_width) {
#define FILL_CASE(W)                                                                                \
    case W: {                                                                                       \
        typename UInt<W>::t v;                                                                      \
        __builtin_memcpy(&v, scalar16, W);                                                          \
        hipLaunchKernelGGL((fill_kernel<typename UInt<W>::t>), dim3(g), dim3(kBlock), 0, s, v, n,   \
                           static_cast<typename UInt<W>::t*>(out));                                 \
    } break;
        FILL_CASE(1) FILL_CASE(2) FILL_CASE(4) FILL_CASE(8) FILL_CASE(16)
#undef FILL_CASE
    default: return VXG_ERR_INVALID_ARGUMENT;
    }
    return hip_check(hipGetLastError(), "fill_kernel");
}

__device__ __forceinline__ uint32_t abyte(uint32_t hi, uint32_t lo, uint32_t sh) {
    return __builtin_amdgcn_alignbyte(hi, lo, sh);
}
template <int QD>
__device__ __forceinline__ uint4 funnel16(const uint4& lo, const uint4& hi, uint32_t rb) {
    const uint32_t w[8] = {lo.x, lo.y, lo.z, lo.w, hi.x, hi.y, hi.z, hi.w};
    return make_uint4(abyte(w[QD + 1], w[QD], rb), abyte(w[QD + 2], w[QD + 1], rb), abyte(w[QD + 3], w[QD + 2], rb),
                      abyte(w[QD + 4], w[QD + 3], rb));
}

__global__ __launch_bounds__(kBlock) void copy_bytes_kernel(uint8_t* __restrict__ dst, const uint8_t* __restrict__ src,
                                                            uint64_t n, uint64_t head, uint64_t body, uint32_t r) {
    const uint64_t stride = uint64_t(gridDim.x) * blockDim.x;
    const uint64_t t0 = uint64_t(blockIdx.x) * blockDim.x + threadIdx.x;
    uint4* const d16 = reinterpret_cast<uint4*>(dst + head);
    if (!src) {
        for (uint64_t q = t0; q < body; q += stride) gstore(d16 + q, make_uint4(0, 0, 0, 0));
    } else if (r == 0) {
        const uint4* const s16 = reinterpret_cast<const uint4*>(src + head);
        for (uint64_t q = t0; q < body; q += stride) gstore(d16 + q, gload(s16 + q));
    } else {
        const uint4* const s16 = reinterpret_cast<const uint4*>(src + head - r);
        const uint32_t qd = r >> 2, rb = r & 3;
        for (uint64_t q = t0; q < body; q += stride) {
            const uint4 lo = gload(s16 + q), hi = gload(s16 + q + 1);
            uint4 v;
            if (qd == 0) v = funnel16<0>(lo, hi, rb);
            else if (qd == 1) v = funnel16<1>(lo, hi, rb);
            else if (qd == 2) v = funnel16<2>(lo, hi, rb);
            else v = funnel16<3>(lo, hi, rb);
            gstore(d16 + q, v);
        }
    }
    const uint64_t tail0 = head + 16 * body, edge = head + (n - tail0);
    for (uint64_t k = t0; k < edge; k += stride) {
        const uint64_t i = k < head ? k : tail0 + (k - head);
        gstore(dst + i, src ? gload(src + i) : uint8_t(0));
    }
}

vxg_status launch_copy_bytes(void* dst, const void* src, uint64_t n, hipStream_t s) {
    if (n == 0) return VXG_OK;
    const uintptr_t d = reinterpret_cast<uintptr_t>(dst), a = reinterpret_cast<uintptr_t>(src);
    const uint64_t head = std::min<uint64_t>(n, (16 - (d & 15)) & 15);
    const uint64_t body = (n - head) / 16;
    const uint32_t r = src ? uint32_t((a + head) & 15) : 0u;
    const uint64_t work = std::max<uint64_t>(body, 32);
    hipLaunchKernelGGL(copy_bytes_kernel, dim3(grid_for(work)), dim3(kBlock), 0, s, static_cast<uint8_t*>(dst),
                       static_cast<const uint8_t*>(src), n, head, body, r);
    return hip_check(hipGetLastError(), "copy_bytes_kernel");
}

__device__ __forceinline__ uint4 make_view(const uint8_t* __restrict__ heap, uint64_t start, uint32_t len,
                                          uint32_t bidx) {
    const uint8_t* p = heap + start;
    uint32_t w1 = 0, w2 = 0, w3 = 0;
    if (len <= 12) {
#pragma unroll
        for (int j = 0; j < 12; j++) {
            const uint32_t b = uint32_t(j) < len ? uint32_t(gload(p + j)) : 0u;
            if (j < 4) w1 |= b << (8 * j);
            else if (j < 8) w2 |= b << (8 * (j - 4));
            else w3 |= b << (8 * (j - 8));
        }
    } else {
#pragma unroll
        for (int j = 0; j < 4; j++) w1 |= uint32_t(gload(p + j)) << (8 * j);
        w2 = bidx;
        w3 = uint32_t(start);
    }
    return make_uint4(len, w1, w2, w3);
}

__device__ __forceinline__ uint4 checked_view(const uint8_t* __restrict__ heap, uint64_t heap_len, uint64_t a,
                                              uint64_t e, uint32_t bidx, uint32_t* err) {
    if (a > e || e > heap_len) {
        __hip_atomic_fetch_or(err, kErrVarBin, __ATOMIC_RELAXED, __HIP_MEMORY_SCOPE_AGENT);
        return make_uint4(0, 0, 0, 0);
    }
    return make_view(heap, a, uint32_t(e - a), bidx);
}

__global__ __launch_bounds__(kBlock) void varbin_views_kernel(const uint8_t* __restrict__ heap, uint64_t heap_len,
                                                              const void* offs, int offs_width, uint64_t n,
                                                              const uint8_t* __restrict__ validity,
                                                              uint32_t bidx, uint4* __restrict__ views, uint32_t* err) {
    const uint64_t stride = uint64_t(gridDim.x) * blockDim.x;
    for (uint64_t i = uint64_t(blockIdx.x) * blockDim.x + threadIdx.x; i < n; i += stride) {
        if (validity && !((validity[i >> 3] >> (i & 7)) & 1)) {
            views[i] = make_uint4(0, 0, 0, 0);
            continue;
        }
        const uint64_t a = load_uint(offs, offs_width, offs_width < 8, i);
        const uint64_t b = load_uint(offs, offs_width, offs_width < 8, i + 1);
        views[i] = checked_view(heap, heap_len, a, b, bidx, err);
    }
}

vxg_status launch_varbin_views(const uint8_t* heap, uint64_t heap_len, int offs_width, const void* offsets, uint64_t n,
                               const uint8_t* validity, uint32_t bidx, uint8_t* views, uint32_t* err, hipStream_t s) {
    if (n == 0) return VXG_OK;
    hipLaunchKernelGGL(varbin_views_kernel, dim3(grid_for(n)), dim3(kBlock), 0, s, heap, heap_len, offsets,
                       offs_width, n, validity, bidx, reinterpret_cast<uint4*>(views), err);
    return hip_check(hipGetLastError(), "varbin_views_kernel");
}

__global__ __launch_bounds__(kBlock) void varbin_chunks_kernel(VarBinTable tab) {
    const uint64_t g = blockIdx.x;
    VarBinChunk c;
    if (tab.ext) {
        c = tab.ext[ext_chunk_index(tab.ext, tab.n, g, [](VarBinChunk const& d) { return d.first_group; })];
    } else {
        uint32_t lo = 0, hi = tab.n;
        while (hi - lo > 1) {
            const uint32_t mid = (lo + hi) >> 1;
            if (tab.c[mid].first_group <= g) lo = mid; else hi = mid;
        }
        c = tab.c[lo];
    }
    const uint64_t lg = g - c.first_group;
    const uint64_t ng = (c.n + kBlock - 1) / kBlock > 0 ? (c.n + kBlock - 1) / kBlock : 1;
    const uint64_t per = (c.bytes + ng - 1) / ng;
    for (uint64_t b = lg * per + threadIdx.x; b < c.bytes && b < (lg + 1) * per; b += kBlock) gstore(c.dst + b, gload(c.src + b));
    const uint64_t i = lg * kBlock + threadIdx.x;
    if (i < c.n) {
        const uint64_t a = load_uint(c.offsets, int(c.offs_width), c.offs_width < 8, i);
        const uint64_t e = load_uint(c.offsets, int(c.offs_width), c.offs_width < 8, i + 1);
        gstore(reinterpret_cast<uint4*>(c.views) + i, checked_view(c.src, c.bytes, a, e, c.bidx, tab.err));
    }
}

vxg_status launch_varbin_chunks(const VarBinTable& t, uint64_t groups, hipStream_t s) {
    if (groups == 0) return VXG_OK;
    hipLaunchKernelGGL(varbin_chunks_kernel, dim3(unsigned(groups)), dim3(kBlock), 0, s, t);
    return hip_check(hipGetLastError(), "varbin_chunks_kernel");
}

__global__ __launch_bounds__(kBlock) void views_rebase_kernel(const uint4* __restrict__ src, uint64_t n, uint32_t add,
                                                              uint4* __restrict__ dst) {
    const uint64_t stride = uint64_t(gridDim.x) * blockDim.x;
    for (uint64_t i = uint64_t(blockIdx.x) * blockDim.x + threadIdx.x; i < n; i += stride) {
        uint4 v = src[i];
        if (v.x > 12) v.z += add;
        dst[i] = v;
    }
}

vxg_status launch_views_rebase(const uint8_t* src, uint64_t n, uint32_t add, uint8_t* dst, hipStream_t s) {
    if (n == 0) return VXG_OK;
    hipLaunchKernelGGL(views_rebase_kernel, dim3(grid_for(n)), dim3(kBlock), 0, s,
                       reinterpret_cast<const uint4*>(src), n, add, reinterpret_cast<uint4*>(dst));
    return hip_check(hipGetLastError(), "views_rebase_kernel");
}

__device__ __forceinline__ void put_bits(uint32_t* __restrict__ dst, uint64_t pos, uint32_t word, bool full) {
    const uint64_t w = pos >> 5;
    const int sh = int(pos & 31);
    if (full && sh == 0) {
        dst[w] = word;
        return;
    }
    if (!word) return;
    atomicOr(dst + w, word << sh);
    if (sh) {
        const uint32_t hi = word >> (32 - sh);
        if (hi) atomicOr(dst + w + 1, hi);
    }
}

constexpr int kBoolSpan = 32 * kBlock;
__global__ __launch_bounds__(kBlock) void runend_bool_kernel(const void* __restrict__ ends, int ew, uint64_t n_runs,
                                                             uint64_t offset, int start, uint64_t len,
                                                             uint32_t* __restrict__ dst, uint64_t dst_off,
                                                             uint32_t* __restrict__ err) {
    __shared__ uint32_t s_flip[kBlock];
    __shared__ uint32_t s_wpar[kBlock / 64];
    __shared__ uint64_t s_r0;
    const int tid = threadIdx.x, lane = tid & 63, wave = tid >> 6;
    const uint64_t j0 = uint64_t(blockIdx.x) * kBoolSpan;
    const uint64_t jend = len - j0 < uint64_t(kBoolSpan) ? len : j0 + kBoolSpan;
    s_flip[tid] = 0;
    if (tid < 64) {
        const uint64_t r0 = runend_first_gt(ends, ew, offset, n_runs, j0);
        if (tid == 0) s_r0 = r0;
        if (blockIdx.x == 0 && tid == 0 && load_uint(ends, ew, false, n_runs - 1) - offset < len)
            __hip_atomic_fetch_or(err, kErrRunEnd, __ATOMIC_RELAXED, __HIP_MEMORY_SCOPE_AGENT);
    }
    __syncthreads();
    const uint64_t r0 = s_r0;
    if (r0 >= n_runs) {
        return;
    }
    for (uint64_t r = r0 + tid; r < n_runs; r += kBlock) {
        const uint64_t e = load_uint(ends, ew, false, r) - offset;
        if (e >= jend) break;
        const uint32_t p = uint32_t(e - j0);
        atomicXor(&s_flip[p >> 5], 1u << (p & 31));
    }
    __syncthreads();
    const uint32_t f = s_flip[tid];
    uint32_t x = f;
    x ^= x << 1;
    x ^= x << 2;
    x ^= x << 4;
    x ^= x << 8;
    x ^= x << 16;
    const unsigned long long bal = __ballot(__popc(f) & 1);
    const uint32_t below = uint32_t(__popcll(bal & ((1ull << lane) - 1ull)) & 1);
    if (lane == 0) s_wpar[wave] = uint32_t(__popcll(bal) & 1);
    __syncthreads();
    uint32_t carry = below ^ uint32_t(start != 0) ^ uint32_t(r0 & 1);
    for (int w = 0; w < wave; w++) carry ^= s_wpar[w];
    uint32_t word = x ^ (carry ? 0xFFFFFFFFu : 0u);
    const uint64_t p0 = j0 + uint64_t(tid) * 32;
    if (p0 >= jend) return;
    const uint64_t nb = jend - p0;
    if (nb < 32) word &= (1u << nb) - 1u;
    put_bits(dst, dst_off + p0, word, nb >= 32);
}

vxg_status launch_runend_bool(const void* ends, int ew, uint64_t n_runs, uint64_t offset, bool start, uint64_t len,
                              void* dst, uint64_t dst_off, uint32_t* err, hipStream_t s) {
    if (len == 0) return VXG_OK;
    if (n_runs == 0) return set_error(VXG_ERR_INVALID_ARGUMENT, "Ends array must have at least one element");
    const uint64_t groups = (len + kBoolSpan - 1) / kBoolSpan;
    if (groups > 0xFFFFFFFFull) return set_error(VXG_ERR_INVALID_ARGUMENT, "RunEndBool too long");
    hipLaunchKernelGGL(runend_bool_kernel, dim3(unsigned(groups)), dim3(kBlock), 0, s, ends, ew, n_runs, offset,
                       int(start), len, static_cast<uint32_t*>(dst), dst_off, err);
    return hip_check(hipGetLastError(), "runend_bool_kernel");
}

__device__ __forceinline__ uint32_t nonzero_nibble(uint32_t v) {
    const uint32_t m = (((v & 0x7F7F7F7Fu) + 0x7F7F7F7Fu) | v) & 0x80808080u;
    const uint32_t b = m >> 7;
    return (b | (b >> 7) | (b >> 14) | (b >> 21)) & 0xFu;
}

__global__ __launch_bounds__(kBlock) void bytebool_kernel(const uint8_t* __restrict__ src, uint64_t n,
                                                          uint32_t* __restrict__ dst, uint64_t dst_off) {
    const uint64_t stride = uint64_t(gridDim.x) * blockDim.x;
    for (uint64_t w = uint64_t(blockIdx.x) * blockDim.x + threadIdx.x; w * 32 < n; w += stride) {
        const uint64_t p0 = w * 32;
        uint32_t word = 0;
        if (p0 + 32 <= n && (reinterpret_cast<uintptr_t>(src + p0) & 15) == 0) {
            const uint4 a = reinterpret_cast<const uint4*>(src + p0)[0];
            const uint4 b = reinterpret_cast<const uint4*>(src + p0)[1];
            const uint32_t q[8] = {a.x, a.y, a.z, a.w, b.x, b.y, b.z, b.w};
#pragma unroll
            for (int k = 0; k < 8; k++) word |= nonzero_nibble(q[k]) << (4 * k);
        } else {
            for (int k = 0; k < 32 && p0 + k < n; k++) word |= uint32_t(src[p0 + k] != 0) << k;
        }
        put_bits(dst, dst_off + p0, word, p0 + 32 <= n);
    }
}

vxg_status launch_bytebool(const uint8_t* src, uint64_t n, void* dst, uint64_t dst_off, hipStream_t s) {
    if (n == 0) return VXG_OK;
    hipLaunchKernelGGL(bytebool_kernel, dim3(grid_for((n + 31) / 32)), dim3(kBlock), 0, s, src, n,
                       static_cast<uint32_t*>(dst), dst_off);
    return hip_check(hipGetLastError(), "bytebool_kernel");
}

__global__ __launch_bounds__(kBlock) void assign_bits_at_kernel(uint32_t* __restrict__ dst, uint64_t dst_off,
                                                                const void* idx, int iw, int isg, uint64_t ioff,
                                                                uint64_t n, uint64_t len,
                                                                const uint8_t* __restrict__ vals) {
    const uint64_t stride = uint64_t(gridDim.x) * blockDim.x;
    for (uint64_t i = uint64_t(blockIdx.x) * blockDim.x + threadIdx.x; i < n; i += stride) {
        const uint64_t p = load_uint(idx, iw, isg != 0, i) - ioff;
        if (p >= len) continue;
        const uint64_t q = dst_off + p;
        const uint32_t bit = 1u << (q & 31);
        if ((vals[i >> 3] >> (i & 7)) & 1) atomicOr(dst + (q >> 5), bit);
        else atomicAnd(dst + (q >> 5), ~bit);
    }
}

vxg_status launch_assign_bits_at(void* dst, uint64_t dst_off, const void* idx, int iw, bool isg, uint64_t ioff,
                                 uint64_t n, uint64_t len, const uint8_t* vals, hipStream_t s) {
    if (n == 0) return VXG_OK;
    hipLaunchKernelGGL(assign_bits_at_kernel, dim3(grid_for(n)), dim3(kBlock), 0, s, static_cast<uint32_t*>(dst),
                       dst_off, idx, iw, int(isg), ioff, n, len, vals);
    return hip_check(hipGetLastError(), "assign_bits_at_kernel");
}

__global__ __launch_bounds__(kBlock) void gather_bits_kernel(uint32_t* __restrict__ dst, const void* codes, int cw,
                                                             bool csg, uint64_t n, const uint8_t* __restrict__ src,
                                                             uint64_t n_values, uint32_t* __restrict__ err) {
    const uint64_t stride = uint64_t(gridDim.x) * blockDim.x;
    for (uint64_t w = uint64_t(blockIdx.x) * blockDim.x + threadIdx.x; w * 32 < n; w += stride) {
        uint32_t word = 0;
        bool oob = false;
        for (int k = 0; k < 32; k++) {
            const uint64_t i = w * 32 + k;
            if (i >= n) break;
            const uint64_t c = load_uint(codes, cw, csg, i);
            oob |= c >= n_values;
            word |= (c < n_values ? uint32_t((src[c >> 3] >> (c & 7)) & 1) : 0u) << k;
        }
        if (oob) __hip_atomic_fetch_or(err, kErrTakeOOB, __ATOMIC_RELAXED, __HIP_MEMORY_SCOPE_AGENT);
        dst[w] = word;
    }
}

vxg_status launch_gather_bits(void* dst, const void* codes, int cw, bool csg, uint64_t n, const uint8_t* src,
                              uint64_t n_values, uint32_t* err, hipStream_t s) {
    if (n == 0) return VXG_OK;
    hipLaunchKernelGGL(gather_bits_kernel, dim3(grid_for((n + 31) / 32)), dim3(kBlock), 0, s,
                       static_cast<uint32_t*>(dst), codes, cw, csg, n, src, n_values, err);
    return hip_check(hipGetLastError(), "gather_bits_kernel");
}

}
```

### vortex_amd/csrc/planner_launch.hip

```cpp
#include <algorithm>
#include <tuple>

#include "chunk_pack.hpp"
#include "k1g.hpp"
#include "planner.hpp"

static_assert(sizeof(vxg::ChunkTable) <= 4096, "ChunkTable exceeds the kernarg limit");
static_assert(sizeof(vxg::FsstTable) <= 4096, "FsstTable exceeds the kernarg limit");
static_assert(sizeof(vxg::RunEndTable) <= 4096, "RunEndTable exceeds the kernarg limit");
static_assert(sizeof(vxg::VarBinTable) <= 4096, "VarBinTable exceeds the kernarg limit");
static_assert(sizeof(vxg::CmpTable) + 32 <= 4096, "CmpTable and the compare arguments exceed the kernarg limit");

namespace vxg {

void note_k1w_launch(uint32_t bpw, uint32_t bpw_max, uint64_t groups) {
    if (!g_cur_ctx) return;
    std::lock_guard<std::mutex> lk(g_cur_ctx->mu);
    LaunchStats& st = g_cur_ctx->st;
    st.k1w_min_bpw = st.k1w_launches == 0 ? bpw : std::min(st.k1w_min_bpw, bpw);
    st.k1w_max_bpw = st.k1w_launches == 0 ? bpw : std::max(st.k1w_max_bpw, bpw);
    st.k1w_launches++;
    st.k1w_last_bpw = bpw;
    st.k1w_last_bpw_max = bpw_max;
    st.k1w_last_groups = groups;
}

vxg_status launch_fl_unpack(int T, int W, Epi epi, int vw, const ChunkTable& t, uint64_t g, hipStream_t s) {
    if (W < 0 || W > T) return set_error(VXG_ERR_INVALID_ARGUMENT, "bit width out of range");
    switch (epi) {
    case Epi::Plain:
    case Epi::For:
    case Epi::ForZigZag:
        switch (T) {
        case 8: return fl_plain_8(W, epi, t, g, s);
        case 16: return fl_plain_16(W, epi, t, g, s);
        case 32: return fl_plain_32(W, epi, t, g, s);
        case 64: return fl_plain_64(W, epi, t, g, s);
        }
        return set_error(VXG_ERR_INVALID_ARGUMENT, "bad FastLanes width");
    case Epi::AlpF32:
    case Epi::AlpF64:
        return fl_alp(T, W, epi, t, g, s);
    case Epi::Dict:
        if (W > kDictFusedMaxW) return VXG_ERR_NOT_IMPLEMENTED;
        switch (vw) {
        case 1: return fl_dict_1(T, W, t, g, s);
        case 2: return fl_dict_2(T, W, t, g, s);
        case 4: return fl_dict_4(T, W, t, g, s);
        case 8: return fl_dict_8(T, W, t, g, s);
        case 16: return launch_dict_rows(T, W, t, s);
        }
        return set_error(VXG_ERR_INVALID_ARGUMENT, "bad dictionary value width");
    }
    return VXG_ERR_INVALID_ARGUMENT;
}

static bool same_kernel(const K1Job& a, const K1Job& b) {
    return a.T == b.T && a.W == b.W && a.epi == b.epi && a.vw == b.vw && a.vb == b.vb;
}

static uint64_t k1g_max_bytes() {
    static const uint64_t v = env_u64("VXG_K1G_MAX_BYTES", uint64_t(20) << 20);
    return v;
}

static int k1_out_width(int T, Epi epi, int vw) {
    return epi == Epi::Dict ? vw : (epi == Epi::AlpF32 ? 4 : (epi == Epi::AlpF64 ? 8 : T / 8));
}

template <class Group>
static vxg_status for_each_kernel_group(std::vector<K1Job>& jobs, size_t max_group, Group group) {
    std::stable_sort(jobs.begin(), jobs.end(), [](const K1Job& a, const K1Job& b) {
        return std::make_tuple(a.T, a.W, int(a.epi), a.vw, a.vb) < std::make_tuple(b.T, b.W, int(b.epi), b.vw, b.vb);
    });
    for (size_t i = 0, j; i < jobs.size(); i = j) {
        uint64_t out_bytes = 0;
        for (j = i; j < jobs.size() && j - i < max_group && same_kernel(jobs[i], jobs[j]); j++)
            out_bytes += jobs[j].d.len * uint64_t(k1_out_width(jobs[j].T, jobs[j].epi, jobs[j].vw));
        VXG_TRY(group(i, j, out_bytes));
    }
    return VXG_OK;
}

static vxg_status launch_kernel_group(const K1Job* it, const K1Job* end, uint32_t* err, hipStream_t s, DevTables* dt,
                                      const PatchCol* patch) {
    const K1Job& k = *it;
    while (it != end) {
        ChunkTable tab{};
        tab.err = err;
        if (patch) tab.patch = *patch;
        uint64_t groups;
        VXG_TRY(pack_chunk_table(
            tab, it, end, dt, [](const K1Job& jb) { return jb.d.n_blocks ? &jb.d : nullptr; },
            [](const ChunkDev& c) { return (c.n_blocks + 31) / 32; }, &groups));
        if (tab.n) VXG_TRY(launch_fl_unpack(k.T, k.W, k.epi, k.vw, tab, groups, s));
    }
    return VXG_OK;
}

static void add_nonempty(std::vector<const K1Job*>& gen, const K1Job* it, const K1Job* end) {
    for (; it != end; ++it)
        if (it->d.n_blocks) gen.push_back(it);
}

vxg_status launch_k1_jobs(std::vector<K1Job>& jobs, uint32_t* err, hipStream_t s, DevTables* dt, const PatchCol* patch) {
    if (patch && jobs.size() != 1) return set_error(VXG_ERR_INVALID_ARGUMENT, "internal: fused patches need a single K1 job");
    std::vector<const K1Job*> gen;
    VXG_TRY(for_each_kernel_group(jobs, dt ? jobs.size() : size_t(kArgChunks), [&](size_t i, size_t j, uint64_t) -> vxg_status {
        if (!jobs[i].vb) return launch_kernel_group(jobs.data() + i, jobs.data() + j, err, s, dt, patch);
        if (!dt) return set_error(VXG_ERR_INVALID_ARGUMENT, "VarBin-dictionary K1 jobs need a plan");
        add_nonempty(gen, jobs.data() + i, jobs.data() + j);
        return VXG_OK;
    }));
    return gen.empty() ? VXG_OK : launch_k1g_jobs(gen, {}, FsstFused{}, err, s, *dt);
}

static vxg_status launch_plan_k1_jobs(std::vector<K1Job>& jobs, const std::vector<std::pair<int, RunEndChunk>>& gen_runs,
                                      const FsstFused& fuse, uint32_t* err, hipStream_t s, DevTables& dt) {
    std::vector<const K1Job*> gen;
    VXG_TRY(for_each_kernel_group(jobs, jobs.size(), [&](size_t i, size_t j, uint64_t out_bytes) -> vxg_status {
        if (const K1Job& k = jobs[i]; !k.vb && (out_bytes >= k1g_max_bytes() || gen_kind(k.T, int(k.epi), k.vw) < 0))
            return launch_kernel_group(jobs.data() + i, jobs.data() + j, err, s, &dt, nullptr);
        add_nonempty(gen, jobs.data() + i, jobs.data() + j);
        return VXG_OK;
    }));
    return launch_k1g_jobs(gen, gen_runs, fuse, err, s, dt);
}

vxg_status make_k1_job(int T, unsigned W, unsigned offset, uint64_t len, const void* packed, uint64_t packed_bytes,
                       Epi epi, int vw, const UnpackArgs& a, void* out, K1Job& j) {
    if (offset > 1023) return set_error(VXG_ERR_INVALID_ARGUMENT, "Offset must be less than full block, i.e. 1024");
    if (W > unsigned(T)) return set_error(VXG_ERR_INVALID_ARGUMENT, "Unsupported bit width");
    const uint64_t nblk = (len + offset + 1023) / 1024;
    if (W > 0 && packed_bytes != nblk * 128ull * W)
        return set_error(VXG_ERR_INVALID_ARGUMENT, "Expected " + std::to_string(nblk * 128ull * W) +
                                                       " packed bytes, got " + std::to_string(packed_bytes));
    if (W > 0 && (reinterpret_cast<uintptr_t>(packed) & 15))
        return set_error(VXG_ERR_INVALID_ARGUMENT, "packed buffer must be 16-byte aligned");
    if (reinterpret_cast<uintptr_t>(out) % uint64_t(k1_out_width(T, epi, vw)))
        return set_error(VXG_ERR_INVALID_ARGUMENT, "output buffer must be aligned to the value width");
    if (epi == Epi::Dict && W > unsigned(kDictFusedMaxW)) return VXG_ERR_NOT_IMPLEMENTED;
    if (epi == Epi::Dict && a.dict_len == 0 && len > 0)
        return set_error(VXG_ERR_OUT_OF_BOUNDS, "take: index out of bounds");
    j.T = T;
    j.W = int(W);
    j.epi = epi;
    j.vw = epi == Epi::Dict ? vw : 0;
    j.d = ChunkDev{};
    j.d.packed = static_cast<const uint8_t*>(packed);
    j.d.out = out;
    j.d.n_blocks = len ? nblk : 0;
    j.d.len = len;
    j.d.reference = a.reference;
    j.d.alp_a = a.alp_a;
    j.d.alp_b = a.alp_b;
    j.d.dict = a.dict;
    j.d.dict_len = a.dict_len;
    j.d.offset = offset;
    j.d.shift = a.shift;
    return VXG_OK;
}

vxg_status launch_runs(std::vector<RunEndChunk> runs, int w, uint32_t* err, hipStream_t s, DevTables* dt) {
    runs.erase(std::remove_if(runs.begin(), runs.end(), [](const RunEndChunk& r) { return r.len == 0; }), runs.end());
    std::vector<RunEndChunk> short_runs, long_runs;
    for (const RunEndChunk& r : runs) (r.len <= kRunEndShortRun * r.n_runs ? short_runs : long_runs).push_back(r);
    for (int pass = 0; pass < 2; pass++) {
        const std::vector<RunEndChunk>& rs = pass == 0 ? short_runs : long_runs;
        for (const RunEndChunk* it = rs.data(), * const end = rs.data() + rs.size(); it != end;) {
            RunEndTable tab{};
            tab.err = err;
            uint64_t groups;
            VXG_TRY(pack_chunk_table(
                tab, it, end, dt, [](const RunEndChunk& r) { return &r; },
                [pass](const RunEndChunk& r) {
                    return pass == 0 ? (r.n_runs + kRunEndRunsPerGroup - 1) / kRunEndRunsPerGroup
                                     : (r.len + kRunEndSpan - 1) / kRunEndSpan;
                },
                &groups));
            VXG_TRY(pass == 0 ? launch_runend_runs(w, tab, groups, s) : launch_runend_chunks(w, tab, groups, s));
        }
    }
    return VXG_OK;
}

static bool plan_fuse_enabled() { return env_flag("VXG_PLAN_FUSE", true); }

vxg_status launch_varbin_dicts(const std::vector<VarBinChunk>& dicts, uint32_t* err, hipStream_t s, DevTables* dt) {
    for (const VarBinChunk* it = dicts.data(), * const end = dicts.data() + dicts.size(); it != end;) {
        VarBinTable tab{};
        tab.err = err;
        uint64_t groups;
        VXG_TRY(pack_chunk_table(
            tab, it, end, dt, [](const VarBinChunk& d) { return &d; },
            [](const VarBinChunk& d) { return d.n ? (d.n + 255) / 256 : uint64_t(1); }, &groups));
        VXG_TRY(launch_varbin_chunks(tab, groups, s));
    }
    return VXG_OK;
}

vxg_status flush_plan_batch(PlanBatch& b, uint32_t* err, hipStream_t s, DevTables* dt) {
    FsstFused ff;
    if (!b.fssts.empty()) {
        void* scratch = nullptr;
        VXG_TRY(hip_check(hipMalloc(&scratch, (fsst_chunks_scratch_bytes(b.fssts.data(), b.fssts.size()) + 15) & ~15ull),
                            "hipMalloc (plan FSST scratch)"));
        dt->allocs.push_back(scratch);
        VXG_TRY(launch_fsst_batch(b.fssts, scratch, err, s, dt, plan_fuse_enabled() ? &ff : nullptr));
    }
    VXG_TRY(launch_varbin_dicts(b.dicts, err, s, dt));
    std::vector<std::pair<int, RunEndChunk>> gen_runs;
    std::vector<PlanBatch::Run> rest;
    for (const PlanBatch::Run& r : b.runs) {
        if (r.c.len == 0) continue;
        if (r.indep && r.c.len <= kRunEndShortRun * r.c.n_runs && gen_runs_kind(r.w) >= 0) gen_runs.emplace_back(r.w, r.c);
        else rest.push_back(r);
    }
    VXG_TRY(launch_plan_k1_jobs(b.jobs, gen_runs, ff, err, s, *dt));
    std::vector<int> widths;
    for (const auto& r : rest) widths.push_back(r.w);
    std::sort(widths.begin(), widths.end());
    widths.erase(std::unique(widths.begin(), widths.end()), widths.end());
    for (int w : widths) {
        std::vector<RunEndChunk> rs;
        for (const auto& r : rest)
            if (r.w == w) rs.push_back(r.c);
        VXG_TRY(launch_runs(rs, w, err, s, dt));
    }
    return VXG_OK;
}

}
```

### vortex_amd/csrc/vxg_internal.hpp

```cpp
#pragma once

#include <hip/hip_runtime.h>

#include <cstdint>
#include <mutex>
#include <string>
#include <type_traits>
#include <vector>

#include "../../include/vortex_gpu.h"
#include "env.hpp"

namespace vxg {

__host__ __device__ constexpr int fl_order(int i) {
    constexpr int o[8] = {0, 4, 2, 6, 1, 5, 3, 7};
    return o[i];
}
__host__ __device__ constexpr int fl_index(int row, int lane) {
    return fl_order(row / 8) * 16 + (row % 8) * 128 + lane;
}

template <class T>
using gptr = __attribute__((address_space(1))) T*;
template <class T>
__device__ __forceinline__ T gload(const T* p) {
    if constexpr (sizeof(T) == 16 && !std::is_scalar_v<T>) {
        using u32x4 = unsigned int __attribute__((ext_vector_type(4)));
        const u32x4 x = *(gptr<const u32x4>)p;
        T r;
        __builtin_memcpy(&r, &x, 16);
        return r;
    } else {
        return *(gptr<const T>)p;
    }
}
template <class T>
__device__ __forceinline__ void gstore(T* p, const T& v) {
    if constexpr (sizeof(T) == 16 && !std::is_scalar_v<T>) {
        using u32x4 = unsigned int __attribute__((ext_vector_type(4)));
        u32x4 x;
        __builtin_memcpy(&x, &v, 16);
        *(gptr<u32x4>)p = x;
    } else {
        *(gptr<T>)p = v;
    }
}
template <class T>
__device__ __forceinline__ T lds_load(const T* p) {
    if constexpr (sizeof(T) == 16 && !std::is_scalar_v<T>) {
        using u32x4 = unsigned int __attribute__((ext_vector_type(4)));
        const u32x4 x = *(__attribute__((address_space(3))) const u32x4*)p;
        T r;
        __builtin_memcpy(&r, &x, 16);
        return r;
    } else {
        return *(__attribute__((address_space(3))) const T*)p;
    }
}

template <typename V>
__device__ __forceinline__ void nt_store(V* p, const V& v) {
    if constexpr (sizeof(V) == 16) {
        using u32x4 = unsigned int __attribute__((ext_vector_type(4)));
        u32x4 vv;
        __builtin_memcpy(&vv, &v, 16);
        __builtin_nontemporal_store(vv, (gptr<u32x4>)p);
    } else {
        __builtin_nontemporal_store(v, (gptr<V>)p);
    }
}

inline int ptype_width(int p) {
    switch (p) {
    case VXG_U8: case VXG_I8: return 1;
    case VXG_U16: case VXG_I16: case VXG_F16: return 2;
    case VXG_U32: case VXG_I32: case VXG_F32: return 4;
    case VXG_U64: case VXG_I64: case VXG_F64: return 8;
    default: return 0;
    }
}
inline bool ptype_is_int(int p) { return p >= VXG_U8 && p <= VXG_I64; }
inline bool ptype_is_signed(int p) { return p >= VXG_I8 && p <= VXG_I64; }
inline bool ptype_is_unsigned(int p) { return p >= VXG_U8 && p <= VXG_U64; }

extern const float kF10f[11];
extern const float kIF10f[11];
extern const double kF10d[24];
extern const double kIF10d[24];

enum : uint32_t { kErrTakeOOB = 1u, kErrPatchOOB = 2u, kErrRunEnd = 4u, kErrFsst = 8u, kErrRoaring = 16u, kErrVarBin = 32u,
                  kErrPatchOrder = 64u, kErrPlanSync = 128u };

struct Options {
    int64_t k1w_min_groups = 1024;
    int64_t k1w_bpw = 0;
    int64_t k1_wave = -1;
};
struct LaunchStats {
    uint64_t k1w_launches = 0, k1w_last_groups = 0;
    uint32_t k1w_last_bpw = 0, k1w_min_bpw = 0, k1w_max_bpw = 0, k1w_last_bpw_max = 0;
};

struct Ctx {
    int device = 0;
    uint32_t* err_word = nullptr;
    Options opt;
    std::mutex mu;
    LaunchStats st;
};
extern thread_local Ctx* g_cur_ctx;
Options default_options();
inline Options cur_options() { return g_cur_ctx ? g_cur_ctx->opt : default_options(); }
inline int k1_wave_mode() {
    const int64_t o = cur_options().k1_wave;
    if (o >= 0) return int(o > 2 ? 2 : o);
    const char* e = env_str("VXG_K1_WAVE");
    if (!e) return 1;
    return e[0] == '0' ? 0 : (e[0] == 'f' ? 2 : 1);
}
void note_k1w_launch(uint32_t bpw, uint32_t bpw_max, uint64_t groups);

vxg_status set_error(vxg_status s, const std::string& msg);
vxg_status hip_check(hipError_t e, const char* what);

struct DevTables {
    std::vector<void*> allocs;
    std::vector<std::pair<void*, std::vector<uint8_t>>> uploads;
    template <class E>
    vxg_status table(size_t n, E** host, const E** dev) {
        void* d = nullptr;
        const hipError_t e = hipMalloc(&d, n * sizeof(E) + 16);
        if (e != hipSuccess) return hip_check(e, "hipMalloc (plan chunk table)");
        allocs.push_back(d);
        uploads.emplace_back(d, std::vector<uint8_t>(n * sizeof(E), 0));
        *host = reinterpret_cast<E*>(uploads.back().second.data());
        *dev = static_cast<const E*>(d);
        return VXG_OK;
    }
    vxg_status upload() {
        for (auto& u : uploads) {
            const hipError_t e = hipMemcpy(u.first, u.second.data(), u.second.size(), hipMemcpyHostToDevice);
            if (e != hipSuccess) return hip_check(e, "plan chunk table upload");
        }
        uploads.clear();
        return VXG_OK;
    }
};

template <class E, class Key>
__device__ __forceinline__ uint32_t ext_chunk_index(const E* __restrict__ ext, uint32_t n, uint64_t g, Key key) {
    const uint32_t lane = threadIdx.x & 63u;
    uint32_t cnt = 0;
    for (uint32_t base = 0; base < n; base += 256) {
        uint64_t kv[4];
#pragma unroll
        for (int k = 0; k < 4; k++) {
            const uint32_t i = base + 64u * uint32_t(k) + lane;
            kv[k] = uint64_t(key(ext[i < n ? i : n - 1]));
        }
#pragma unroll
        for (int k = 0; k < 4; k++) {
            const bool le = base + 64u * uint32_t(k) + lane < n && kv[k] <= g;
            cnt += uint32_t(__popcll(__ballot(le)));
        }
    }
    return cnt ? cnt - 1 : 0;
}

template <class E, class Key>
__device__ __forceinline__ uint32_t ext_chunk_index_gpe(const E* __restrict__ ext, uint32_t n, uint64_t g, uint64_t gpe,
                                                        Key key) {
    if (gpe) {
        const uint32_t q = uint32_t(g) / uint32_t(gpe);
        const uint32_t ci = __builtin_amdgcn_readfirstlane(q < n - 1 ? q : n - 1);
        const uint64_t f0 = uint64_t(key(ext[ci]));
        const uint64_t f1 = ci + 1 < n ? uint64_t(key(ext[ci + 1])) : ~0ull;
        if (f0 <= g && g < f1) return ci;
    }
    return ext_chunk_index(ext, n, g, key);
}
inline uint64_t common_groups(const uint64_t* counts, size_t n) {
    if (n == 0 || counts[0] == 0) return 0;
    for (size_t i = 1; i + 1 < n; i++)
        if (counts[i] != counts[0]) return 0;
    return counts[n - 1] <= counts[0] ? counts[0] : 0;
}

enum class Epi : int { Plain = 0, For = 1, ForZigZag = 2, AlpF32 = 3, AlpF64 = 4, Dict = 5 };

struct UnpackArgs {
    const uint8_t* packed;
    void* out;
    uint64_t n_blocks;
    uint32_t offset;
    uint64_t len;
    uint64_t reference;
    uint32_t shift;
    double alp_a, alp_b;
    const void* dict;
    uint64_t dict_len;
    uint32_t* err;
};

struct ChunkDev {
    const uint8_t* packed;
    void* out;
    uint64_t n_blocks;
    uint64_t len;
    uint64_t first_group;
    uint64_t reference;
    double alp_a, alp_b;
    const void* dict;
    uint64_t dict_len;
    uint32_t offset;
    uint32_t shift;
};
constexpr int kArgChunks = 32;
struct ChunkTable;

vxg_status launch_fl_unpack(int T, int W, Epi epi, int value_width, const ChunkTable& tab, uint64_t groups,
                            hipStream_t s);

struct IntCol {
    const void* p;
    int width;
    bool sgn;
    bool packed;
    uint32_t W;
    uint32_t shift;
    uint32_t offset;
    uint64_t reference;
};
struct PatchCol {
    IntCol idx;
    const void* vals;
    uint64_t n;
    uint64_t idx_off;
};

struct ChunkTable {
    ChunkDev c[kArgChunks];
    uint32_t n;
    uint32_t* err;
    const ChunkDev* ext;
    ChunkDev* host;
    PatchCol patch;
    uint32_t bpw;
};

inline uint64_t split_below_groups() {
    static const uint64_t v = env_u64("VXG_SPLIT_BELOW", 1024);
    return v;
}

enum class K1Kind { None, Reg, RegSplit, Wave };
struct K1Choice { K1Kind kind; bool lds; };
inline K1Choice k1_choose(int T, int W, Epi epi, bool is_ext, uint64_t groups32, bool lds_ok, int mode,
                          uint64_t split_below) {
    if (groups32 == 0) return {K1Kind::None, false};
    const bool can_split = (T == 32 || T == 64) && W > 0;
    const bool split = can_split && groups32 < split_below;
    constexpr uint64_t kExtWaveGroups = 128;
    const bool big = !split || (is_ext && groups32 >= kExtWaveGroups);
    const bool lds = epi == Epi::Dict && lds_ok;
    if (mode == 2 || (mode == 1 && big && epi != Epi::Dict)) return {K1Kind::Wave, lds};
    return {(is_ext ? can_split : split) ? K1Kind::RegSplit : K1Kind::Reg, lds};
}

vxg_status launch_patch(int val_width, const IntCol& indices, Epi epi, int T, void* out, uint64_t out_len,
                        uint64_t indices_offset, const void* values, uint64_t n, const UnpackArgs& ep,
                        hipStream_t s);

vxg_status launch_for(int width, const void* in, uint64_t n, uint64_t ref, unsigned shift,
                      bool zigzag, void* out, hipStream_t s);
vxg_status launch_zigzag(int width, const void* in, uint64_t n, void* out, hipStream_t s);
vxg_status launch_alp(int float_ptype, const void* enc, uint64_t n, double a, double b, void* out,
                      hipStream_t s);
vxg_status launch_take(int value_width, const void* values, uint64_t n_values, int code_width, bool code_signed,
                       const void* codes, uint64_t n, void* out, uint32_t* err, hipStream_t s);
vxg_status launch_alprd(int float_ptype, const uint16_t* left, const uint16_t* dict, unsigned dict_len,
                        unsigned right_bw, const void* right, uint64_t n, const void* exc_pos,
                        int pos_width, bool pos_signed, uint64_t pos_off, const uint16_t* exc,
                        uint64_t n_exc, void* out, uint32_t* err, hipStream_t s);
vxg_status launch_copy_bits(void* dst, uint64_t dst_off, const uint8_t* src, uint64_t src_off, uint64_t n,
                            bool set_all, hipStream_t s);
vxg_status launch_roaring_bool(const uint8_t* buf, uint64_t n, uint64_t len, void* bits, uint64_t off, uint32_t* err,
                               hipStream_t s);
vxg_status launch_runend_bool(const void* ends, int ew, uint64_t n_runs, uint64_t offset, bool start, uint64_t len,
                              void* dst, uint64_t dst_off, uint32_t* err, hipStream_t s);
vxg_status launch_bytebool(const uint8_t* src, uint64_t n, void* dst, uint64_t dst_off, hipStream_t s);
vxg_status launch_assign_bits_at(void* dst, uint64_t dst_off, const void* idx, int iw, bool isg, uint64_t ioff,
                                 uint64_t n, uint64_t len, const uint8_t* vals, hipStream_t s);
vxg_status launch_gather_bits(void* dst, const void* codes, int cw, bool csg, uint64_t n, const uint8_t* src,
                              uint64_t n_values, uint32_t* err, hipStream_t s);
vxg_status launch_set_bits_at(void* dst, const void* idx, int iw, bool isg, uint64_t off, uint64_t n,
                              uint64_t len, hipStream_t s);
vxg_status launch_sum(const void* p, int w, bool sg, uint64_t n, void* out_u64, hipStream_t s);
vxg_status fl_plain_8(int W, Epi epi, const ChunkTable& t, uint64_t g, hipStream_t s);
vxg_status fl_plain_16(int W, Epi epi, const ChunkTable& t, uint64_t g, hipStream_t s);
vxg_status fl_plain_32(int W, Epi epi, const ChunkTable& t, uint64_t g, hipStream_t s);
vxg_status fl_plain_64(int W, Epi epi, const ChunkTable& t, uint64_t g, hipStream_t s);
vxg_status fl_alp(int T, int W, Epi epi, const ChunkTable& t, uint64_t g, hipStream_t s);
vxg_status launch_dict_rows(int T, int W, const ChunkTable& tab, hipStream_t s);
#define VXG_DECL_DICT(VW) vxg_status fl_dict_##VW(int T, int W, const ChunkTable& t, uint64_t g, hipStream_t s);
VXG_DECL_DICT(1)
VXG_DECL_DICT(2)
VXG_DECL_DICT(4)
VXG_DECL_DICT(8)
#undef VXG_DECL_DICT
constexpr int kDictFusedMaxW = 16;
vxg_status launch_delta(int width, const void* bases, const void* deltas, uint64_t n_deltas,
                        uint64_t offset, uint64_t len, void* out, hipStream_t s);
struct RunEndChunk {
    IntCol ends;
    IntCol values;
    void* out;
    uint64_t n_runs;
    uint64_t offset;
    uint64_t len;
    uint64_t first_group;
};
vxg_status launch_runend(int value_width, const RunEndChunk& chunk, uint32_t* err, hipStream_t s);
constexpr uint64_t kRunEndSpan = 4096;
constexpr int kRunEndArgChunks = 32;
struct RunEndTable {
    RunEndChunk c[kRunEndArgChunks];
    uint32_t n;
    uint32_t* err;
    const RunEndChunk* ext;
};
vxg_status launch_runend_chunks(int value_width, const RunEndTable& t, uint64_t groups, hipStream_t s);
constexpr uint64_t kRunEndShortRun = 16;
constexpr uint64_t kRunEndRunsPerGroup = 1024;
vxg_status launch_runend_runs(int value_width, const RunEndTable& t, uint64_t groups, hipStream_t s);

struct VarBinChunk {
    const uint8_t* src;
    uint8_t* dst;
    const void* offsets;
    uint8_t* views;
    uint64_t bytes;
    uint64_t n;
    uint64_t first_group;
    uint32_t offs_width;
    uint32_t bidx;
};
constexpr int kVarBinArgChunks = 48;
struct VarBinTable {
    VarBinChunk c[kVarBinArgChunks];
    uint32_t n;
    const VarBinChunk* ext;
    uint32_t* err;
};
vxg_status launch_varbin_chunks(const VarBinTable& t, uint64_t groups, hipStream_t s);

vxg_status launch_copy_bytes(void* dst, const void* src, uint64_t n, hipStream_t s);
vxg_status launch_fill(int value_width, const uint8_t* scalar16, uint64_t n, void* out,
                       hipStream_t s);
struct FsstChunk {
    const uint64_t* symbols;
    const uint8_t* sym_lens;
    const uint8_t* codes;
    const uint8_t* validity;
    uint8_t* heap;
    uint8_t* views;
    IntCol offs;
    IntCol lens;
    uint64_t n;
    uint64_t heap_len;
    uint64_t first_tile;
    uint64_t first_scan;
    uint32_t n_symbols;
    uint32_t bidx;
};
constexpr int kFsstArgChunks = 24;
struct FsstTable {
    FsstChunk c[kFsstArgChunks];
    uint32_t n;
    const FsstChunk* ext;
};
uint64_t fsst_scratch_bytes(uint64_t n);
uint64_t fsst_chunks_scratch_bytes(const FsstChunk* chunks, size_t n_chunks);
struct FsstFusedArgs {
    const FsstChunk* ext;
    const int64_t* tp;
    const int64_t* bt;
    const int64_t* tc;
    const uint32_t* wg_chunk;
    uint64_t tiles;
    uint64_t mix;
    uint64_t prepass;
    uint64_t delay;
    const uint32_t* scan_chunk;
    uint32_t tag;
};
bool is_fsst_fused_kernel(const void* func);
struct FsstFused {
    bool valid = false;
    int oa = 0, la = 0;
    FsstFusedArgs a{};
};
hipError_t fsst_diag_init();
vxg_status launch_fsst_batch(std::vector<FsstChunk>& chunks, void* scratch, uint32_t* err, hipStream_t s,
                             DevTables* dt = nullptr, FsstFused* fuse = nullptr);
vxg_status launch_varbin_views(const uint8_t* heap, uint64_t heap_len, int offs_width, const void* offsets, uint64_t n,
                               const uint8_t* validity, uint32_t bidx, uint8_t* views, uint32_t* err, hipStream_t s);
vxg_status launch_views_rebase(const uint8_t* src, uint64_t n, uint32_t add, uint8_t* dst, hipStream_t s);

}
```

Baseline: 4898.

## Pack chunk tables into compact kernel arguments to cut launch count

Adds a compact 40-byte per-chunk argument format, plus a packed VarBin format, so up to 96 K1 chunks (92 VarBin chunks) fit in the kernel-argument block. Previously the limit was 32 (48 for VarBin), after which work split into more launches or needed a device table. Kernels expand the compact entries on device and recompute block counts and ALP factors from small indices. It also adds launch counters and an option to cap compact chunk length. The cost is extra per-block decode work and host-side packing checks. For a single large u32 column this may rarely trigger.

```diff
diff --git a/vortex_amd/arrays.py b/vortex_amd/arrays.py
--- a/vortex_amd/arrays.py
+++ b/vortex_amd/arrays.py
@@ -457,7 +457,8 @@
         _lib.check(self.lib.vxg_stream_sync(self.handle, self.stream_ptr()))
 
     _OPTIONS = {"k1w_min_groups": _lib.OPT_K1W_MIN_GROUPS, "k1w_bpw": _lib.OPT_K1W_BPW,
-                "k1_wave": _lib.OPT_K1_WAVE}
+                "k1_wave": _lib.OPT_K1_WAVE,
+                "compact_max_len": 1000, "k1_launches": 1001, "runend_launches": 1002, "varbin_launches": 1003}
 
     def set_option(self, name: str, value: int):
         _lib.check(self.lib.vxg_set_option(self.handle, self._OPTIONS[name], int(value)))
diff --git a/vortex_amd/csrc/capi.hip b/vortex_amd/csrc/capi.hip
--- a/vortex_amd/csrc/capi.hip
+++ b/vortex_amd/csrc/capi.hip
@@ -128,6 +128,10 @@
         if (value < -1 || value > 2) return set_error(VXG_ERR_INVALID_ARGUMENT, "K1_WAVE must be -1, 0, 1 or 2");
         o.k1_wave = value;
         return VXG_OK;
+    case kOptCompactMaxLen:
+        if (value < 0 || value > 0xFFFFFFFFll) return set_error(VXG_ERR_INVALID_ARGUMENT, "compact chunk length limit out of range");
+        o.compact_max_len = value;
+        return VXG_OK;
     }
     return set_error(VXG_ERR_INVALID_ARGUMENT, "unknown option " + std::to_string(option));
 }
@@ -139,6 +143,16 @@
     case VXG_OPT_K1W_MIN_GROUPS: *value = o.k1w_min_groups; return VXG_OK;
     case VXG_OPT_K1W_BPW: *value = o.k1w_bpw; return VXG_OK;
     case VXG_OPT_K1_WAVE: *value = o.k1_wave; return VXG_OK;
+    case kOptCompactMaxLen: *value = o.compact_max_len; return VXG_OK;
+    case kOptK1Launches:
+    case kOptRunEndLaunches:
+    case kOptVarBinLaunches: {
+        std::lock_guard<std::mutex> lk(ctx->c.mu);
+        const LaunchStats& st = ctx->c.st;
+        *value = int64_t(option == kOptK1Launches ? st.k1_launches
+                                                  : (option == kOptRunEndLaunches ? st.runend_launches : st.varbin_launches));
+        return VXG_OK;
+    }
     }
     return set_error(VXG_ERR_INVALID_ARGUMENT, "unknown option " + std::to_string(option));
 }
diff --git a/vortex_amd/csrc/chunk_arg.hpp b/vortex_amd/csrc/chunk_arg.hpp
--- /dev/null
+++ b/vortex_amd/csrc/chunk_arg.hpp
@@ -0,0 +1,199 @@
+#pragma once
+
+#include <cstdint>
+#include <cstring>
+
+#if defined(__HIPCC__)
+#define VXG_HD __host__ __device__
+#else
+#define VXG_HD
+#endif
+
+namespace vxg {
+
+enum class Epi : int { Plain = 0, For = 1, ForZigZag = 2, AlpF32 = 3, AlpF64 = 4, Dict = 5 };
+
+struct ChunkDev {
+    const uint8_t* packed;
+    void* out;
+    uint64_t n_blocks;
+    uint64_t len;
+    uint64_t first_group;
+    uint64_t reference;
+    double alp_a, alp_b;
+    const void* dict;
+    uint64_t dict_len;
+    uint32_t offset;
+    uint32_t shift;
+};
+
+struct ChunkArg {
+    const uint8_t* packed;
+    void* out;
+    uint64_t ref;
+    uint32_t len;
+    uint32_t first_group;
+    uint32_t aux;
+    uint16_t offset;
+    uint8_t shift;
+    uint8_t pad;
+};
+static_assert(sizeof(ChunkArg) == 40, "ChunkArg is 40 bytes");
+constexpr int kArgChunksCompact = 96;
+
+template <bool F32>
+VXG_HD inline double alp_f10(uint32_t f) {
+    if constexpr (F32) {
+        constexpr float t[11] = {1.0f, 10.0f, 100.0f, 1000.0f, 10000.0f, 100000.0f, 1000000.0f,
+                                 10000000.0f, 100000000.0f, 1000000000.0f, 10000000000.0f};
+        return f < 11 ? double(t[f]) : 0.0;
+    } else {
+        constexpr double t[24] = {
+            1.0, 10.0, 100.0, 1000.0, 10000.0, 100000.0, 1000000.0, 10000000.0, 100000000.0,
+            1000000000.0, 10000000000.0, 100000000000.0, 1000000000000.0, 10000000000000.0,
+            100000000000000.0, 1000000000000000.0, 10000000000000000.0, 100000000000000000.0,
+            1000000000000000000.0, 10000000000000000000.0, 100000000000000000000.0,
+            1000000000000000000000.0, 10000000000000000000000.0, 100000000000000000000000.0};
+        return f < 24 ? t[f] : 0.0;
+    }
+}
+template <bool F32>
+VXG_HD inline double alp_if10(uint32_t e) {
+    if constexpr (F32) {
+        constexpr float t[11] = {1.0f, 0.1f, 0.01f, 0.001f, 0.0001f, 0.00001f, 0.000001f,
+                                 0.0000001f, 0.00000001f, 0.000000001f, 0.0000000001f};
+        return e < 11 ? double(t[e]) : 0.0;
+    } else {
+        constexpr double t[24] = {
+            1.0, 0.1, 0.01, 0.001, 0.0001, 0.00001, 0.000001, 0.0000001, 0.00000001, 0.000000001,
+            0.0000000001, 0.00000000001, 0.000000000001, 0.0000000000001, 0.00000000000001,
+            0.000000000000001, 0.0000000000000001, 0.00000000000000001, 0.000000000000000001,
+            0.0000000000000000001, 0.00000000000000000001, 0.000000000000000000001,
+            0.0000000000000000000001, 0.00000000000000000000001};
+        return e < 24 ? t[e] : 0.0;
+    }
+}
+
+VXG_HD inline uint64_t chunk_blocks(uint64_t len, uint32_t offset) {
+    return len ? (len + offset + 1023) >> 10 : 0;
+}
+
+template <bool F32, bool INV>
+inline int alp_exponent_of(double x) {
+    for (uint32_t i = 0; i < (F32 ? 11u : 24u); i++) {
+        const double t = INV ? alp_if10<F32>(i) : alp_f10<F32>(i);
+        if (std::memcmp(&t, &x, sizeof(double)) == 0) return int(i);
+    }
+    return -1;
+}
+
+inline bool pack_chunk_arg(const ChunkDev& c, Epi epi, ChunkArg* a) {
+    if (c.len > 0xFFFFFFFFull || c.first_group > 0xFFFFFFFFull || c.offset > 1023u || c.shift > 255u) return false;
+    if (c.n_blocks != chunk_blocks(c.len, c.offset)) return false;
+    ChunkArg r{};
+    r.packed = c.packed;
+    r.out = c.out;
+    r.len = uint32_t(c.len);
+    r.first_group = uint32_t(c.first_group);
+    r.offset = uint16_t(c.offset);
+    r.shift = uint8_t(c.shift);
+    const bool alp = epi == Epi::AlpF32 || epi == Epi::AlpF64;
+    if (!alp && (c.alp_a != 0.0 || c.alp_b != 0.0)) return false;
+    if (epi == Epi::Dict) {
+        if (c.dict_len > 0xFFFFFFFFull || c.reference != 0) return false;
+        r.ref = uint64_t(reinterpret_cast<uintptr_t>(c.dict));
+        r.aux = uint32_t(c.dict_len);
+    } else {
+        if (c.dict != nullptr || c.dict_len != 0) return false;
+        r.ref = c.reference;
+        if (alp) {
+            const bool f32 = epi == Epi::AlpF32;
+            const int f = f32 ? alp_exponent_of<true, false>(c.alp_a) : alp_exponent_of<false, false>(c.alp_a);
+            const int e = f32 ? alp_exponent_of<true, true>(c.alp_b) : alp_exponent_of<false, true>(c.alp_b);
+            if (f < 0 || e < 0) return false;
+            r.aux = uint32_t(f) | uint32_t(e) << 8;
+        }
+    }
+    *a = r;
+    return true;
+}
+
+template <Epi EPI>
+VXG_HD inline ChunkDev expand_chunk_arg(const ChunkArg& a) {
+    ChunkDev c{};
+    c.packed = a.packed;
+    c.out = a.out;
+    c.len = a.len;
+    c.n_blocks = chunk_blocks(a.len, a.offset);
+    c.first_group = a.first_group;
+    c.offset = a.offset;
+    c.shift = a.shift;
+    if constexpr (EPI == Epi::Dict) {
+        c.dict = reinterpret_cast<const void*>(uintptr_t(a.ref));
+        c.dict_len = a.aux;
+    } else {
+        c.reference = a.ref;
+        if constexpr (EPI == Epi::AlpF32 || EPI == Epi::AlpF64) {
+            c.alp_a = alp_f10<EPI == Epi::AlpF32>(a.aux & 0xFFu);
+            c.alp_b = alp_if10<EPI == Epi::AlpF32>(a.aux >> 8);
+        }
+    }
+    return c;
+}
+
+struct VarBinChunk {
+    const uint8_t* src;
+    uint8_t* dst;
+    const void* offsets;
+    uint8_t* views;
+    uint64_t bytes;
+    uint64_t n;
+    uint64_t first_group;
+    uint32_t offs_width;
+    uint32_t bidx;
+};
+struct __attribute__((packed, aligned(4))) VarBinArg {
+    const uint8_t* src;
+    uint8_t* dst;
+    const void* offsets;
+    uint8_t* views;
+    uint32_t bytes;
+    uint32_t n_ow;
+    uint16_t first_group;
+    uint16_t bidx;
+};
+static_assert(sizeof(VarBinArg) == 44, "VarBinArg is 44 bytes");
+constexpr int kVarBinArgChunksCompact = 92;
+
+inline bool pack_varbin_arg(const VarBinChunk& c, VarBinArg* a) {
+    if (c.bytes > 0xFFFFFFFFull || c.n > 0xFFFFFFull || c.first_group > 0xFFFFull || c.offs_width > 0xFFu ||
+        c.bidx > 0xFFFFu)
+        return false;
+    VarBinArg r{};
+    r.src = c.src;
+    r.dst = c.dst;
+    r.offsets = c.offsets;
+    r.views = c.views;
+    r.bytes = uint32_t(c.bytes);
+    r.n_ow = uint32_t(c.n) | c.offs_width << 24;
+    r.first_group = uint16_t(c.first_group);
+    r.bidx = uint16_t(c.bidx);
+    *a = r;
+    return true;
+}
+
+VXG_HD inline VarBinChunk expand_varbin_arg(const VarBinArg& a) {
+    VarBinChunk c{};
+    c.src = a.src;
+    c.dst = a.dst;
+    c.offsets = a.offsets;
+    c.views = a.views;
+    c.bytes = a.bytes;
+    c.n = a.n_ow & 0xFFFFFFu;
+    c.first_group = a.first_group;
+    c.offs_width = a.n_ow >> 24;
+    c.bidx = a.bidx;
+    return c;
+}
+
+}
diff --git a/vortex_amd/csrc/chunk_pack.hpp b/vortex_amd/csrc/chunk_pack.hpp
--- a/vortex_amd/csrc/chunk_pack.hpp
+++ b/vortex_amd/csrc/chunk_pack.hpp
@@ -2,13 +2,28 @@
 
 #include <algorithm>
 #include <type_traits>
+#include <vector>
 
 #include "vxg_internal.hpp"
 
 namespace vxg {
 
-template <class Tab, class It, class Entry, class Groups>
-vxg_status pack_chunk_table(Tab& tab, It& it, It end, DevTables* dt, Entry entry, Groups groups_of, uint64_t* groups) {
+template <class E, class Fits>
+struct WideTable {
+    std::vector<E>* store;
+    size_t cap;
+    Fits fits;
+};
+template <class Pack>
+struct InlineCompact {
+    bool enabled;
+    Pack pack;
+};
+struct NoWideTable {};
+
+template <class Tab, class It, class Entry, class Groups, class Wide = NoWideTable>
+vxg_status pack_chunk_table(Tab& tab, It& it, It end, DevTables* dt, Entry entry, Groups groups_of, uint64_t* groups,
+                            Wide wide = Wide{}) {
     using E = std::remove_reference_t<decltype(tab.c[0])>;
     constexpr size_t cap = sizeof(tab.c) / sizeof(tab.c[0]);
     size_t take = 0;
@@ -22,7 +37,52 @@
         if constexpr (requires { tab.host; }) tab.host = host;
         cs = host;
     } else {
-        take = std::min(take, cap);
+        size_t share = std::min(take, cap);
+        if constexpr (requires { tab.a; wide.pack; }) {
+            if (take > cap && wide.enabled) {
+                using A = std::remove_reference_t<decltype(tab.a[0])>;
+                constexpr size_t cap_a = sizeof(tab.a) / sizeof(tab.a[0]);
+                const size_t n = std::min(take, cap_a);
+                A packed[cap_a];
+                size_t seen = 0;
+                uint64_t g = 0;
+                bool ok = true;
+                It k = it;
+                for (; k != end && seen < n; ++k)
+                    if (const E* e = entry(*k)) {
+                        E c = *e;
+                        c.first_group = g;
+                        g += groups_of(c);
+                        ok = ok && wide.pack(c, &packed[seen]);
+                        seen++;
+                    }
+                if (ok && g <= 0xFFFFFFFFull) {
+                    std::copy(packed, packed + n, tab.a);
+                    tab.compact = 1;
+                    tab.n = uint32_t(n);
+                    *groups = g;
+                    for (it = k; it != end && !entry(*it);) ++it;
+                    return VXG_OK;
+                }
+            }
+        } else if constexpr (!std::is_same_v<Wide, NoWideTable>) {
+            if (take > cap && wide.store) {
+                const size_t n = std::min(take, wide.cap);
+                size_t seen = 0;
+                bool ok = true;
+                for (It k = it; k != end && seen < n; ++k)
+                    if (const E* e = entry(*k)) {
+                        ok = ok && wide.fits(*e);
+                        seen++;
+                    }
+                if (ok) {
+                    wide.store->assign(n, E{});
+                    tab.host = cs = wide.store->data();
+                    share = n;
+                }
+            }
+        }
+        take = share;
     }
     tab.n = 0;
     *groups = 0;
diff --git a/vortex_amd/csrc/dict_rows.hip b/vortex_amd/csrc/dict_rows.hip
--- a/vortex_amd/csrc/dict_rows.hip
+++ b/vortex_amd/csrc/dict_rows.hip
@@ -11,23 +11,22 @@
 template <> struct DVal<16> { using t = uint4; };
 
 template <int T, int VW, int BPW, bool LDSD, bool EXT>
-__global__ __launch_bounds__(kRowsThreads) void dict_rows_kernel(ChunkTable tab, unsigned W) {
+__global__ __launch_bounds__(kRowsThreads) void dict_rows_kernel(K1Table<EXT> tab, unsigned W) {
     using E = typename Fl<T>::E;
     using V = typename DVal<VW>::t;
     constexpr unsigned LANES = 1024 / T;
     const uint64_t g = blockIdx.x;
-    uint32_t ci;
+    ChunkDev c;
     if constexpr (EXT) {
-        ci = ext_chunk_index(tab.ext, tab.n, g, [](const ChunkDev& d) { return d.first_group; });
+        c = ext_chunk<Epi::Dict>(tab, g);
     } else {
         uint32_t lo = 0, hi = tab.n;
         while (hi - lo > 1) {
             const uint32_t mid = (lo + hi) >> 1;
             if (tab.c[mid].first_group <= g) lo = mid; else hi = mid;
         }
-        ci = lo;
+        c = tab.c[lo];
     }
-    const ChunkDev& c = EXT ? tab.ext[ci] : tab.c[ci];
     __shared__ __attribute__((aligned(16))) E s_packed[BPW * 128 * kRowsMaxW / sizeof(E)];
     __shared__ __attribute__((aligned(16))) uint8_t s_dict[LDSD ? kDictLdsBytes : 16];
     const unsigned tid = threadIdx.x;
@@ -66,7 +65,7 @@
 
 template <int T, int VW, int BPW, bool LDSD, bool EXT>
 vxg_status launch_rows(ChunkTable tab, unsigned W, hipStream_t s) {
-    ChunkDev* cs = tab.ext ? tab.host : tab.c;
+    ChunkDev* cs = host_entries(tab);
     uint64_t groups = 0;
     for (uint32_t k = 0; k < tab.n; k++) {
         cs[k].first_group = groups;
@@ -74,20 +73,27 @@
     }
     if (groups == 0) return VXG_OK;
     if (groups > 0xFFFFFFFFull) return set_error(VXG_ERR_INVALID_ARGUMENT, "array too long for one launch");
-    hipLaunchKernelGGL((dict_rows_kernel<T, VW, BPW, LDSD, EXT>), dim3(unsigned(groups)), dim3(kRowsThreads), 0, s,
-                       tab, W);
+    if constexpr (EXT) {
+        const vxg_status st = launch_table_x(reinterpret_cast<const void*>(&dict_rows_kernel<T, VW, BPW, LDSD, true>), tab,
+                                             Epi::Dict, unsigned(groups), kRowsThreads, 0, s, &W);
+        if (st != VXG_OK) return st;
+    } else {
+        hipLaunchKernelGGL((dict_rows_kernel<T, VW, BPW, LDSD, false>), dim3(unsigned(groups)), dim3(kRowsThreads), 0, s,
+                           tab, W);
+    }
+    note_table_launch(&LaunchStats::k1_launches);
     return hip_check(hipGetLastError(), "dict_rows_kernel launch");
 }
 
 template <int T, int VW, int BPW>
 vxg_status launch_rows_b(const ChunkTable& tab, unsigned W, bool lds, hipStream_t s) {
-    if (tab.ext) return lds ? launch_rows<T, VW, BPW, true, true>(tab, W, s) : launch_rows<T, VW, BPW, false, true>(tab, W, s);
+    if (tab.host) return lds ? launch_rows<T, VW, BPW, true, true>(tab, W, s) : launch_rows<T, VW, BPW, false, true>(tab, W, s);
     return lds ? launch_rows<T, VW, BPW, true, false>(tab, W, s) : launch_rows<T, VW, BPW, false, false>(tab, W, s);
 }
 
 template <int T, int VW>
 vxg_status launch_rows_t(const ChunkTable& tab, unsigned W, hipStream_t s) {
-    const ChunkDev* cs = tab.ext ? tab.host : tab.c;
+    const ChunkDev* cs = host_entries(tab);
     bool lds = true;
     uint64_t max_dict = 0;
     for (uint32_t k = 0; k < tab.n; k++) {
diff --git a/vortex_amd/csrc/fl_unpack_impl.hpp b/vortex_amd/csrc/fl_unpack_impl.hpp
--- a/vortex_amd/csrc/fl_unpack_impl.hpp
+++ b/vortex_amd/csrc/fl_unpack_impl.hpp
@@ -610,12 +610,26 @@
     }
 }
 
+template <bool EXT> struct K1Tab { using t = ChunkTable; };
+template <> struct K1Tab<true> { using t = ChunkTableX; };
+template <bool EXT> using K1Table = typename K1Tab<EXT>::t;
+
+template <Epi EPI>
+__device__ __forceinline__ ChunkDev ext_chunk(const ChunkTableX& tab, uint64_t g) {
+    if (tab.ext) return tab.ext[ext_chunk_index(tab.ext, tab.n, g, [](const ChunkDev& d) { return d.first_group; })];
+    uint32_t lo = 0, hi = tab.n;
+    while (hi - lo > 1) {
+        const uint32_t mid = (lo + hi) >> 1;
+        if (tab.a[mid].first_group <= g) lo = mid; else hi = mid;
+    }
+    return expand_chunk_arg<EPI>(tab.a[lo]);
+}
+
 template <int T, int W, Epi EPI, int VW, bool LDSD, bool EXT>
-__global__ __launch_bounds__(256) void fl_unpack_w_kernel(ChunkTable tab) {
+__global__ __launch_bounds__(256) void fl_unpack_w_kernel(K1Table<EXT> tab) {
     const uint64_t g = blockIdx.x;
     if constexpr (EXT) {
-        const ChunkDev& c =
-            tab.ext[ext_chunk_index(tab.ext, tab.n, g, [](const ChunkDev& d) { return d.first_group; })];
+        const ChunkDev c = ext_chunk<EPI>(tab, g);
         unpack_chunk_w<T, W, EPI, VW, LDSD>(c, g, tab.err, PatchCol{}, tab.bpw);
     } else {
         uint32_t lo = 0, hi = tab.n;
@@ -628,11 +642,10 @@
 }
 
 template <int T, int W, Epi EPI, int VW, bool LDSD = false, int S = 1, bool EXT = false>
-__global__ __launch_bounds__(256) void fl_unpack_kernel(ChunkTable tab) {
+__global__ __launch_bounds__(256) void fl_unpack_kernel(K1Table<EXT> tab) {
     const uint64_t g = blockIdx.x;
     if constexpr (EXT) {
-        const ChunkDev& c =
-            tab.ext[ext_chunk_index(tab.ext, tab.n, g, [](const ChunkDev& d) { return d.first_group; })];
+        const ChunkDev c = ext_chunk<EPI>(tab, g);
         unpack_chunk<T, W, EPI, VW, LDSD, S>(c, g, tab.err);
     } else {
         uint32_t lo = 0, hi = tab.n;
@@ -656,7 +669,7 @@
 template <int T, int W, Epi EPI, int VW, bool LDSD, bool EXT>
 vxg_status launch_w(ChunkTable tab, hipStream_t s) {
     constexpr int BPW_MAX = kw_bpw(W, LDSD);
-    ChunkDev* cs = tab.ext ? tab.host : tab.c;
+    ChunkDev* cs = host_entries(tab);
     uint64_t blocks = 0;
     for (uint32_t k = 0; k < tab.n; k++) blocks += cs[k].n_blocks;
     const Options o = cur_options();
@@ -673,15 +686,22 @@
     if (groups > 0xFFFFFFFFull) return set_error(VXG_ERR_INVALID_ARGUMENT, "array too long for one launch");
     const size_t shm = LDSD ? size_t(kw_packed_lds<W, LDSD>()) + size_t(dict_bytes)
                             : size_t(W > 0 ? BPW * 128 * W : 0) + 128;
-    hipLaunchKernelGGL((fl_unpack_w_kernel<T, W, EPI, VW, LDSD, EXT>), dim3(unsigned(groups)), dim3(256), shm, s, tab);
+    if constexpr (EXT) {
+        const vxg_status st = launch_table_x(reinterpret_cast<const void*>(&fl_unpack_w_kernel<T, W, EPI, VW, LDSD, true>), tab,
+                                             EPI, unsigned(groups), 256, shm, s);
+        if (st != VXG_OK) return st;
+    } else {
+        hipLaunchKernelGGL((fl_unpack_w_kernel<T, W, EPI, VW, LDSD, false>), dim3(unsigned(groups)), dim3(256), shm, s, tab);
+    }
     note_k1w_launch(uint32_t(BPW), uint32_t(BPW_MAX), groups);
+    note_table_launch(&LaunchStats::k1_launches);
     return hip_check(hipGetLastError(), "fl_unpack_w_kernel launch");
 }
 
 
 template <int T, int W, Epi EPI, int VW, bool LDSD, int S, bool EXT = false>
 vxg_status launch_s(ChunkTable tab, hipStream_t s) {
-    ChunkDev* cs = tab.ext ? tab.host : tab.c;
+    ChunkDev* cs = host_entries(tab);
     uint64_t groups = 0;
     for (uint32_t k = 0; k < tab.n; k++) {
         cs[k].first_group = groups;
@@ -689,7 +709,14 @@
     }
     if (groups == 0) return VXG_OK;
     if (groups > 0xFFFFFFFFull) return set_error(VXG_ERR_INVALID_ARGUMENT, "array too long for one launch");
-    hipLaunchKernelGGL((fl_unpack_kernel<T, W, EPI, VW, LDSD, S, EXT>), dim3(unsigned(groups)), dim3(256), 0, s, tab);
+    if constexpr (EXT) {
+        const vxg_status st = launch_table_x(reinterpret_cast<const void*>(&fl_unpack_kernel<T, W, EPI, VW, LDSD, S, true>), tab,
+                                             EPI, unsigned(groups), 256, 0, s);
+        if (st != VXG_OK) return st;
+    } else {
+        hipLaunchKernelGGL((fl_unpack_kernel<T, W, EPI, VW, LDSD, S, false>), dim3(unsigned(groups)), dim3(256), 0, s, tab);
+    }
+    note_table_launch(&LaunchStats::k1_launches);
     return hip_check(hipGetLastError(), "fl_unpack_kernel launch");
 }
 
@@ -698,18 +725,19 @@
     constexpr bool kSplit = (T == 32 || T == 64) && W > 0;
     bool lds_ok = false;
     if constexpr (EPI == Epi::Dict) {
-        const ChunkDev* cs = tab.ext ? tab.host : tab.c;
+        const ChunkDev* cs = host_entries(tab);
         lds_ok = true;
         for (uint32_t k = 0; k < tab.n; k++)
             lds_ok = lds_ok && cs[k].dict_len * VW <= uint64_t(kDictLdsBytes) &&
                      (reinterpret_cast<uintptr_t>(cs[k].dict) & 15) == 0;
     }
-    const K1Choice c = k1_choose(T, W, EPI, tab.ext != nullptr, groups32, lds_ok, k1_wave_mode(), split_below_groups());
+    const bool ext = tab.host != nullptr;
+    const K1Choice c = k1_choose(T, W, EPI, ext, groups32, lds_ok, k1_wave_mode(), split_below_groups());
     const bool wave = c.kind == K1Kind::Wave;
-    if (tab.patch.n && (!wave || tab.ext))
+    if (tab.patch.n && (!wave || ext))
         return set_error(VXG_ERR_INVALID_ARGUMENT, "internal: patches handed to a K1 launch that does not write them");
     if (c.kind == K1Kind::None) return VXG_OK;
-    if (tab.ext) {
+    if (ext) {
         if (wave) {
             if constexpr (EPI == Epi::Dict) {
                 if (c.lds) return launch_w<T, W, EPI, VW, true, true>(tab, s);
diff --git a/vortex_amd/csrc/kernels.hip b/vortex_amd/csrc/kernels.hip
--- a/vortex_amd/csrc/kernels.hip
+++ b/vortex_amd/csrc/kernels.hip
@@ -793,6 +793,13 @@
     VarBinChunk c;
     if (tab.ext) {
         c = tab.ext[ext_chunk_index(tab.ext, tab.n, g, [](VarBinChunk const& d) { return d.first_group; })];
+    } else if (tab.compact) {
+        uint32_t lo = 0, hi = tab.n;
+        while (hi - lo > 1) {
+            const uint32_t mid = (lo + hi) >> 1;
+            if (tab.a[mid].first_group <= g) lo = mid; else hi = mid;
+        }
+        c = expand_varbin_arg(tab.a[lo]);
     } else {
         uint32_t lo = 0, hi = tab.n;
         while (hi - lo > 1) {
diff --git a/vortex_amd/csrc/planner_launch.hip b/vortex_amd/csrc/planner_launch.hip
--- a/vortex_amd/csrc/planner_launch.hip
+++ b/vortex_amd/csrc/planner_launch.hip
@@ -6,6 +6,7 @@
 #include "planner.hpp"
 
 static_assert(sizeof(vxg::ChunkTable) <= 4096, "ChunkTable exceeds the kernarg limit");
+static_assert(sizeof(vxg::ChunkTableX) + 8 <= 4096, "ChunkTableX (and K14's bit width) exceeds the kernarg limit");
 static_assert(sizeof(vxg::FsstTable) <= 4096, "FsstTable exceeds the kernarg limit");
 static_assert(sizeof(vxg::RunEndTable) <= 4096, "RunEndTable exceeds the kernarg limit");
 static_assert(sizeof(vxg::VarBinTable) <= 4096, "VarBinTable exceeds the kernarg limit");
@@ -23,6 +24,31 @@
     st.k1w_last_bpw = bpw;
     st.k1w_last_bpw_max = bpw_max;
     st.k1w_last_groups = groups;
+}
+
+void note_table_launch(uint64_t LaunchStats::*counter) {
+    if (!g_cur_ctx) return;
+    std::lock_guard<std::mutex> lk(g_cur_ctx->mu);
+    (g_cur_ctx->st.*counter)++;
+}
+
+vxg_status make_table_x(const ChunkTable& tab, Epi epi, ChunkTableX& x) {
+    x.n = tab.n;
+    x.bpw = tab.bpw;
+    x.err = tab.err;
+    x.ext = tab.ext;
+    if (tab.ext) return VXG_OK;
+    bool ok = tab.host && tab.n <= uint32_t(kArgChunksCompact);
+    for (uint32_t k = 0; ok && k < tab.n; k++) ok = pack_chunk_arg(tab.host[k], epi, &x.a[k]);
+    return ok ? VXG_OK : set_error(VXG_ERR_INVALID_ARGUMENT, "internal: chunk does not fit the compact table");
+}
+
+vxg_status launch_table_x(const void* kernel, const ChunkTable& tab, Epi epi, unsigned groups, unsigned threads, size_t shm,
+                          hipStream_t s, unsigned* extra) {
+    ChunkTableX x;
+    VXG_TRY(make_table_x(tab, epi, x));
+    void* args[2] = {&x, extra};
+    return hip_check(hipLaunchKernel(kernel, dim3(groups), dim3(threads), args, shm, s), "K1 launch (device or compact table)");
 }
 
 vxg_status launch_fl_unpack(int T, int W, Epi epi, int vw, const ChunkTable& t, uint64_t g, hipStream_t s) {
@@ -85,6 +111,17 @@
 static vxg_status launch_kernel_group(const K1Job* it, const K1Job* end, uint32_t* err, hipStream_t s, DevTables* dt,
                                       const PatchCol* patch) {
     const K1Job& k = *it;
+    std::vector<ChunkDev> wide_store;
+    const Epi epi = k.epi;
+    const uint64_t max_len = uint64_t(cur_options().compact_max_len);
+    const auto fits = [epi, max_len](const ChunkDev& c) {
+        if (c.len > max_len) return false;
+        ChunkDev d = c;
+        d.first_group = 0;
+        ChunkArg a;
+        return pack_chunk_arg(d, epi, &a);
+    };
+    const bool compact = !patch && max_len != 0;
     while (it != end) {
         ChunkTable tab{};
         tab.err = err;
@@ -92,7 +129,8 @@
         uint64_t groups;
         VXG_TRY(pack_chunk_table(
             tab, it, end, dt, [](const K1Job& jb) { return jb.d.n_blocks ? &jb.d : nullptr; },
-            [](const ChunkDev& c) { return (c.n_blocks + 31) / 32; }, &groups));
+            [](const ChunkDev& c) { return (c.n_blocks + 31) / 32; }, &groups,
+            WideTable<ChunkDev, decltype(fits)>{compact ? &wide_store : nullptr, size_t(kArgChunksCompact), fits}));
         if (tab.n) VXG_TRY(launch_fl_unpack(k.T, k.W, k.epi, k.vw, tab, groups, s));
     }
     return VXG_OK;
@@ -106,7 +144,8 @@
 vxg_status launch_k1_jobs(std::vector<K1Job>& jobs, uint32_t* err, hipStream_t s, DevTables* dt, const PatchCol* patch) {
     if (patch && jobs.size() != 1) return set_error(VXG_ERR_INVALID_ARGUMENT, "internal: fused patches need a single K1 job");
     std::vector<const K1Job*> gen;
-    VXG_TRY(for_each_kernel_group(jobs, dt ? jobs.size() : size_t(kArgChunks), [&](size_t i, size_t j, uint64_t) -> vxg_status {
+    const size_t max_group = dt || cur_options().compact_max_len != 0 ? jobs.size() : size_t(kArgChunks);
+    VXG_TRY(for_each_kernel_group(jobs, max_group, [&](size_t i, size_t j, uint64_t) -> vxg_status {
         if (!jobs[i].vb) return launch_kernel_group(jobs.data() + i, jobs.data() + j, err, s, dt, patch);
         if (!dt) return set_error(VXG_ERR_INVALID_ARGUMENT, "VarBin-dictionary K1 jobs need a plan");
         add_nonempty(gen, jobs.data() + i, jobs.data() + j);
@@ -179,6 +218,7 @@
                 },
                 &groups));
             VXG_TRY(pass == 0 ? launch_runend_runs(w, tab, groups, s) : launch_runend_chunks(w, tab, groups, s));
+            if (groups) note_table_launch(&LaunchStats::runend_launches);
         }
     }
     return VXG_OK;
@@ -187,14 +227,18 @@
 static bool plan_fuse_enabled() { return env_flag("VXG_PLAN_FUSE", true); }
 
 vxg_status launch_varbin_dicts(const std::vector<VarBinChunk>& dicts, uint32_t* err, hipStream_t s, DevTables* dt) {
+    const auto pack = [](const VarBinChunk& c, VarBinArg* a) { return pack_varbin_arg(c, a); };
+    const bool compact = cur_options().compact_max_len != 0;
     for (const VarBinChunk* it = dicts.data(), * const end = dicts.data() + dicts.size(); it != end;) {
         VarBinTable tab{};
         tab.err = err;
         uint64_t groups;
         VXG_TRY(pack_chunk_table(
             tab, it, end, dt, [](const VarBinChunk& d) { return &d; },
-            [](const VarBinChunk& d) { return d.n ? (d.n + 255) / 256 : uint64_t(1); }, &groups));
+            [](const VarBinChunk& d) { return d.n ? (d.n + 255) / 256 : uint64_t(1); }, &groups,
+            InlineCompact<decltype(pack)>{compact, pack}));
         VXG_TRY(launch_varbin_chunks(tab, groups, s));
+        if (groups) note_table_launch(&LaunchStats::varbin_launches);
     }
     return VXG_OK;
 }
diff --git a/vortex_amd/csrc/vxg_internal.hpp b/vortex_amd/csrc/vxg_internal.hpp
--- a/vortex_amd/csrc/vxg_internal.hpp
+++ b/vortex_amd/csrc/vxg_internal.hpp
@@ -9,6 +9,7 @@
 #include <vector>
 
 #include "../../include/vortex_gpu.h"
+#include "chunk_arg.hpp"
 #include "env.hpp"
 
 namespace vxg {
@@ -96,10 +97,14 @@
     int64_t k1w_min_groups = 1024;
     int64_t k1w_bpw = 0;
     int64_t k1_wave = -1;
-};
+    int64_t compact_max_len = 0xFFFFFFFFll;
+};
+enum : int { kOptCompactMaxLen = 1000, kOptK1Launches = 1001, kOptRunEndLaunches = 1002, kOptVarBinLaunches = 1003 };
 struct LaunchStats {
     uint64_t k1w_launches = 0, k1w_last_groups = 0;
     uint32_t k1w_last_bpw = 0, k1w_min_bpw = 0, k1w_max_bpw = 0, k1w_last_bpw_max = 0;
+    uint64_t k1_launches = 0;
+    uint64_t runend_launches = 0, varbin_launches = 0;
 };
 
 struct Ctx {
@@ -120,6 +125,7 @@
     return e[0] == '0' ? 0 : (e[0] == 'f' ? 2 : 1);
 }
 void note_k1w_launch(uint32_t bpw, uint32_t bpw_max, uint64_t groups);
+void note_table_launch(uint64_t LaunchStats::*counter);
 
 vxg_status set_error(vxg_status s, const std::string& msg);
 vxg_status hip_check(hipError_t e, const char* what);
@@ -187,7 +193,6 @@
     return counts[n - 1] <= counts[0] ? counts[0] : 0;
 }
 
-enum class Epi : int { Plain = 0, For = 1, ForZigZag = 2, AlpF32 = 3, AlpF64 = 4, Dict = 5 };
 
 struct UnpackArgs {
     const uint8_t* packed;
@@ -203,19 +208,6 @@
     uint32_t* err;
 };
 
-struct ChunkDev {
-    const uint8_t* packed;
-    void* out;
-    uint64_t n_blocks;
-    uint64_t len;
-    uint64_t first_group;
-    uint64_t reference;
-    double alp_a, alp_b;
-    const void* dict;
-    uint64_t dict_len;
-    uint32_t offset;
-    uint32_t shift;
-};
 constexpr int kArgChunks = 32;
 struct ChunkTable;
 
@@ -248,6 +240,18 @@
     PatchCol patch;
     uint32_t bpw;
 };
+struct ChunkTableX {
+    ChunkArg a[kArgChunksCompact];
+    uint32_t n;
+    uint32_t bpw;
+    uint32_t* err;
+    const ChunkDev* ext;
+};
+inline ChunkDev* host_entries(ChunkTable& t) { return t.host ? t.host : t.c; }
+inline const ChunkDev* host_entries(const ChunkTable& t) { return t.host ? t.host : t.c; }
+vxg_status make_table_x(const ChunkTable& tab, Epi epi, ChunkTableX& x);
+vxg_status launch_table_x(const void* kernel, const ChunkTable& tab, Epi epi, unsigned groups, unsigned threads, size_t shm,
+                          hipStream_t s, unsigned* extra = nullptr);
 
 inline uint64_t split_below_groups() {
     static const uint64_t v = env_u64("VXG_SPLIT_BELOW", 1024);
@@ -335,21 +339,14 @@
 constexpr uint64_t kRunEndRunsPerGroup = 1024;
 vxg_status launch_runend_runs(int value_width, const RunEndTable& t, uint64_t groups, hipStream_t s);
 
-struct VarBinChunk {
-    const uint8_t* src;
-    uint8_t* dst;
-    const void* offsets;
-    uint8_t* views;
-    uint64_t bytes;
-    uint64_t n;
-    uint64_t first_group;
-    uint32_t offs_width;
-    uint32_t bidx;
-};
 constexpr int kVarBinArgChunks = 48;
 struct VarBinTable {
-    VarBinChunk c[kVarBinArgChunks];
+    union {
+        VarBinChunk c[kVarBinArgChunks];
+        VarBinArg a[kVarBinArgChunksCompact];
+    };
     uint32_t n;
+    uint32_t compact;
     const VarBinChunk* ext;
     uint32_t* err;
 };
```

Measured after the change: 4888. About the same (-0.2%).
